# AMReX-Fluids/IAMR

Measured on AMD Instinct MI355X. Metric: cells-advanced/sec, higher is better.
Workload: dtype f64; 1 GPU; TaylorGreen 3D single level, one 256^3 box per GPU in a 1x1x1 arrangement (256x256x256 cells), periodic, nu=1e-4 cfl=0.7 Godunov_PLM be_cn_theta=0.5, full NavierStokes::advance per step

## Files before the change

iamr_amd/csrc/cabi.hip:

```cpp
#include "../../include/iamrx.h"
#include "operators.h"
#include "launch.h"
#include "amrns.h"
#include <string>
#include <cstring>
#include <vector>
#include <map>

using namespace iamrx;

struct iamrx_layout_s { LayoutP p; };
struct iamrx_mf_s { MultiFab mf; };

static thread_local std::string g_err;

#define IAMRX_TRY try {
#define IAMRX_CATCH                                                   \
    return 0; }                                                       \
    catch (const std::exception& e) { g_err = e.what(); return 1; }   \
    catch (...) { g_err = "unknown error"; return 2; }

static Geometry to_geom(const iamrx_geom* g)
{
    Geometry r;
// ... 452 lines not shown
            tb[d].define(phi->mf.layout, face_type(d), 3, 0);
            tensor_bcoef(tb[d], *b[d], d);
            b[d] = &tb[d];
        }
        mg.setTensor(true);
    }
    mg.setBCoeffs(b);
    mg.prepare();
    MGStats s = mg.solve(phi->mf, rhs->mf, rtol, atol);
    from_stats(s, st);
    IAMRX_CATCH
}

int iamrx_mlmg_mac_solve(const iamrx_geom* g, iamrx_mf ux, iamrx_mf uy, iamrx_mf uz, iamrx_mf rho, int rho_comp, iamrx_mf S,
                         iamrx_mf mac_phi, double rhs_scale, const int lobc[3], const int hibc[3], double mac_tol,
                         double mac_abs_tol, const iamrx_mg_opts* o, iamrx_mg_stats* st)
{
    IAMRX_TRY
    MGOpts op = to_opts(o);
    MultiFab* um[3] = {&ux->mf, &uy->mf, &uz->mf};
    MGStats s = mlmg_mac_solve(to_geom(g), um, rho->mf, rho_comp, S ? &S->mf : nullptr, mac_phi->mf, rhs_scale,
                               to_bc(lobc, hibc, op.maxorder), mac_tol, mac_abs_tol, op, nullptr);
    from_stats(s, st);
    IAMRX_CATCH
}

int iamrx_mlmg_mac_solve_cf(const iamrx_geom* g, iamrx_mf ux, iamrx_mf uy, iamrx_mf uz, iamrx_mf rho, int rho_comp, iamrx_mf S,
                            iamrx_mf mac_phi, double rhs_scale, const int lobc[3], const int hibc[3], iamrx_mf crse_phi,
                            const iamrx_geom* cgeom, int ratio, double mac_tol, double mac_abs_tol, const iamrx_mg_opts* o, iamrx_mg_stats* st)
{
    IAMRX_TRY
    IAMRX_ASSERT(ratio == 2 && cgeom);
    MGOpts op = to_opts(o);
    MultiFab* um[3] = {&ux->mf, &uy->mf, &uz->mf};
    const Geometry cg = to_geom(cgeom);
    MGStats s = mlmg_mac_solve(to_geom(g), um, rho->mf, rho_comp, S ? &S->mf : nullptr, mac_phi->mf, rhs_scale,
                               to_bc(lobc, hibc, op.maxorder), mac_tol, mac_abs_tol, op, nullptr, crse_phi ? &crse_phi->mf : nullptr, &cg, ratio);
    from_stats(s, st);
    IAMRX_CATCH
}

int iamrx_derive_mag_vort(const iamrx_geom* g, iamrx_mf out, int ocomp, iamrx_mf vel, int vcomp)
{
    IAMRX_TRY derive_mag_vort(to_geom(g), out->mf, ocomp, vel->mf, vcomp); IAMRX_CATCH
}

int iamrx_error_tag(const iamrx_geom* g, iamrx_mf tags, iamrx_mf field, int comp, int mode, double value, int level,
                    const double* realbox_lo, const double* realbox_hi)
{
    IAMRX_TRY error_tag(to_geom(g), tags->mf, field->mf, comp, mode, value, level, realbox_lo, realbox_hi); IAMRX_CATCH
}

int iamrx_host_cluster_tags(const unsigned char* tags, const int dom_lo[3], const int dom_hi[3], int blocking_factor, int max_grid_size, double grid_eff,
                            int n_error_buf, const unsigned char* allowed, int* boxes, int* nboxes)
{
    IAMRX_TRY
    BoxD dom;
    for (int d = 0; d < 3; ++d) { dom.lo[d] = dom_lo[d]; dom.hi[d] = dom_hi[d]; }
    std::vector<BoxD> bx = cluster_tags(tags, dom, blocking_factor, max_grid_size, grid_eff, n_error_buf, nullptr, allowed);
    if ((int)bx.size() > *nboxes) throw Error("iamrx_host_cluster_tags: box capacity too small");
    *nboxes = (int)bx.size();
    for (size_t q = 0; q < bx.size(); ++q) for (int d = 0; d < 3; ++d) { boxes[6 * q + d] = bx[q].lo[d]; boxes[6 * q + 3 + d] = bx[q].hi[d]; }
    IAMRX_CATCH
}
int iamrx_host_erode(unsigned char* map, const int n[3], const int periodic[3], int passes)
{
    IAMRX_TRY
    std::vector<unsigned char> m(map, map + (size_t)n[0] * n[1] * n[2]);
    int lo[3] = {n[0], n[1], n[2]}, hi[3] = {-1, -1, -1};
    for (int k = 0; k < n[2]; ++k) for (int j = 0; j < n[1]; ++j) for (int i = 0; i < n[0]; ++i)
        if (m[((size_t)k * n[1] + j) * n[0] + i]) { const int c[3] = {i, j, k}; for (int d = 0; d < 3; ++d) { lo[d] = std::min(lo[d], c[d]); hi[d] = std::max(hi[d], c[d]); } }
    erode_map(m, n, periodic, passes, lo, hi);
    std::copy(m.begin(), m.end(), map);
    IAMRX_CATCH
}
int iamrx_cluster_tags(const iamrx_geom* g, iamrx_mf tags, int blocking_factor, int max_grid_size, double grid_eff, int n_error_buf,
                       int* boxes, int* nboxes)
{
    IAMRX_TRY
    const Geometry gg = to_geom(g);
    const MultiFab& T = tags->mf;
    IAMRX_ASSERT(Context::get().comm->nranks == 1);
    const int n0 = gg.domain.len(0), n1 = gg.domain.len(1), n2 = gg.domain.len(2);
    std::vector<unsigned char> h((size_t)n0 * n1 * n2, 0);
    for (int li = 0; li < T.nlocal(); ++li) {
        const BoxD fb = T.fabbox(li);
        std::vector<double> buf((size_t)fb.npts() * T.ncomp);
        T.copy_to_host(li, buf.data());
        const BoxD vb = T.layout->lbox(li);
        for (int k = vb.lo[2]; k <= vb.hi[2]; ++k) for (int j = vb.lo[1]; j <= vb.hi[1]; ++j) for (int i = vb.lo[0]; i <= vb.hi[0]; ++i) {
            const size_t o = ((size_t)(k - fb.lo[2]) * fb.len(1) + (j - fb.lo[1])) * fb.len(0) + (i - fb.lo[0]);
            if (buf[o] != 0.0) h[((size_t)(k - gg.domain.lo[2]) * n1 + (j - gg.domain.lo[1])) * n0 + (i - gg.domain.lo[0])] = 1;
        }
    }
    std::vector<BoxD> bx = cluster_tags(h.data(), gg.domain, blocking_factor, max_grid_size, grid_eff, n_error_buf);
    if ((int)bx.size() > *nboxes) throw Error("iamrx_cluster_tags: box capacity too small");
    *nboxes = (int)bx.size();
    for (size_t q = 0; q < bx.size(); ++q) for (int d = 0; d < 3; ++d) { boxes[6 * q + d] = bx[q].lo[d]; boxes[6 * q + 3 + d] = bx[q].hi[d]; }
    IAMRX_CATCH
}

int iamrx_mac_divergence(const iamrx_geom* g, iamrx_mf div, iamrx_mf ux, iamrx_mf uy, iamrx_mf uz)
{
    IAMRX_TRY
    const MultiFab* um[3] = {&ux->mf, &uy->mf, &uz->mf};
    mac_divergence(to_geom(g), div->mf, um);
    IAMRX_CATCH
}

static std::vector<BCRec> to_bcrec(const int* b, int n)
{
    std::vector<BCRec> r(n);
    for (int i = 0; i < n; ++i)
        for (int d = 0; d < 3; ++d) { r[i].lo[d] = b ? b[6 * i + d] : 0; r[i].hi[d] = b ? b[6 * i + 3 + d] : 0; }
    return r;
}

int iamrx_mf_fill_physbc(iamrx_mf m, const iamrx_geom* g, int scomp, int ncomp, const int* bcrec, const double* edlo, const double* edhi)
{
    IAMRX_TRY
    auto bc = to_bcrec(bcrec, ncomp);
    fill_physbc_cc(to_geom(g), m->mf, scomp, ncomp, bc.data(), edlo, edhi);
    IAMRX_CATCH
}

int iamrx_godunov_extrap_vel_to_faces(const iamrx_geom* g, iamrx_mf vel, iamrx_mf force, iamrx_mf ux, iamrx_mf uy, iamrx_mf uz,
                                      double dt, const int* bcrec, int fit, int scheme)
{
    IAMRX_TRY
    auto bc = to_bcrec(bcrec, 3);
    MultiFab* um[3] = {&ux->mf, &uy->mf, &uz->mf};
    godunov_extrap_vel_to_faces(to_geom(g), vel->mf, force ? &force->mf : nullptr, um, dt, bc.data(), fit != 0, scheme);
    IAMRX_CATCH
}

int iamrx_godunov_compute_aofs(const iamrx_geom* g, iamrx_mf aofs, int acomp, iamrx_mf S, int ncomp, iamrx_mf force, iamrx_mf divu,
                               iamrx_mf ux, iamrx_mf uy, iamrx_mf uz, const int* iconserv, double dt, const int* bcrec,
                               int is_velocity, int fit, iamrx_mf ex, iamrx_mf ey, iamrx_mf ez, iamrx_mf fx, iamrx_mf fy, iamrx_mf fz, int scheme)
{
    IAMRX_TRY
    auto bc = to_bcrec(bcrec, ncomp);
    MultiFab* um[3] = {&ux->mf, &uy->mf, &uz->mf};
    MultiFab* ed[3] = {ex ? &ex->mf : nullptr, ey ? &ey->mf : nullptr, ez ? &ez->mf : nullptr};
    MultiFab* fl[3] = {fx ? &fx->mf : nullptr, fy ? &fy->mf : nullptr, fz ? &fz->mf : nullptr};
    godunov_compute_aofs(to_geom(g), aofs->mf, acomp, S->mf, ncomp, force ? &force->mf : nullptr, divu ? &divu->mf : nullptr, um,
                         iconserv, dt, bc.data(), is_velocity != 0, fit != 0, ex ? ed : nullptr, fx ? fl : nullptr, scheme);
    IAMRX_CATCH
}

int iamrx_nodal_residual(const iamrx_geom* g, iamrx_mf out, iamrx_mf phi, iamrx_mf sig, iamrx_mf rhs)
{
    IAMRX_TRY nodal_residual(to_geom(g), out->mf, phi->mf, sig->mf, rhs ? &rhs->mf : nullptr); IAMRX_CATCH
}
int iamrx_nodal_gs_color(const iamrx_geom* g, iamrx_mf phi, iamrx_mf rhs, iamrx_mf sig, int color)
{
    IAMRX_TRY nodal_gs_color(to_geom(g), phi->mf, rhs->mf, sig->mf, color); IAMRX_CATCH
}
int iamrx_nodal_gs_sweep(const iamrx_geom* g, iamrx_mf phi, iamrx_mf rhs, iamrx_mf sig, int fused)
{
    IAMRX_TRY
    Geometry gg = to_geom(g);
    if (fused == 3 || fused == 4) {
        static MultiFab& xb = *new MultiFab();
        if (!xb.defined() || xb.layout != phi->mf.layout || xb.ngrow != phi->mf.ngrow) xb.define(phi->mf.layout, node_type(), 1, phi->mf.ngrow);
        const bool wrap = fused == 4;
        if (wrap && !periodic_wrap_ok(gg, *phi->mf.layout, 4)) throw Error("iamrx_nodal_gs_sweep(4): not a single box spanning a periodic domain");
        const double cs = tune("BENCH_CSIG", 0.0);
        nodal_gs_fused_pass(gg, phi->mf, phi->mf, xb, rhs->mf, sig->mf, 0, wrap, nullptr, cs != 0.0 ? &cs : nullptr);
        nodal_gs_fused_pass(gg, phi->mf, xb, xb, rhs->mf, sig->mf, 1, wrap, nullptr, cs != 0.0 ? &cs : nullptr);
    } else if (fused == 2) {
        if (!nodal_smooth_small(gg, phi->mf, rhs->mf, sig->mf, 1)) throw Error("level does not qualify for the single-workgroup smoother");
        phi->mf.FillBoundary(gg);
    } else if (fused) {
        MultiFab xb(phi->mf.layout, node_type(), 1, phi->mf.ngrow);
        phi->mf.FillBoundary(gg);
        nodal_gs_fused_pass(gg, phi->mf, phi->mf, xb, rhs->mf, sig->mf, 0);
        xb.FillBoundary(gg);
        nodal_gs_fused_pass(gg, phi->mf, xb, xb, rhs->mf, sig->mf, 1);
        MultiFab::Copy(phi->mf, xb, 0, 0, 1, 0);
    } else {
        for (int c = 0; c < 8; ++c) { phi->mf.FillBoundary(gg); nodal_gs_color(gg, phi->mf, rhs->mf, sig->mf, c); }
    }
    IAMRX_CATCH
}
int iamrx_nodal_restrict(iamrx_mf c, iamrx_mf f) { IAMRX_TRY nodal_restrict(c->mf, f->mf); IAMRX_CATCH }
int iamrx_nodal_interp_add(iamrx_mf f, iamrx_mf c, iamrx_mf s) { IAMRX_TRY nodal_interp_add(f->mf, c->mf, s->mf); IAMRX_CATCH }
int iamrx_nodal_divu(const iamrx_geom* g, iamrx_mf rhs, iamrx_mf vel, int vcomp)
{
    IAMRX_TRY
    Geometry gg = to_geom(g);
    DomainBC bc;
    for (int d = 0; d < 3; ++d) bc.lo[d] = bc.hi[d] = gg.periodic[d] ? lo_periodic : lo_neumann;
    bc.maxorder = 2;
    nodal_divu(gg, rhs->mf, vel->mf, vcomp, &bc);
    IAMRX_CATCH
}
int iamrx_nodal_divu_bc(const iamrx_geom* g, iamrx_mf rhs, iamrx_mf vel, int vcomp, const int lobc[3], const int hibc[3])
{
    IAMRX_TRY
    const DomainBC bc = to_bc(lobc, hibc, 2);
    nodal_divu(to_geom(g), rhs->mf, vel->mf, vcomp, &bc);
    IAMRX_CATCH
}
int iamrx_nodal_compgrad(const iamrx_geom* g, iamrx_mf gp, iamrx_mf phi)
{
    IAMRX_TRY nodal_mknewu(to_geom(g), nullptr, 0, phi->mf, nullptr, &gp->mf, false); IAMRX_CATCH
}

int iamrx_nodal_projection(const iamrx_geom* g, iamrx_mf vel, int vcomp, iamrx_mf phi, iamrx_mf sig, int sig_comp, const int lobc[3],
                           const int hibc[3], double rel_tol, double abs_tol, const iamrx_mg_opts* o, iamrx_mf gp, int increment_gp,
                           iamrx_mg_stats* st)
{
    IAMRX_TRY
    MGOpts op = to_opts(o);
    MGStats s = nodal_projection(to_geom(g), vel->mf, vcomp, phi->mf, sig->mf, sig_comp, to_bc(lobc, hibc, op.maxorder), rel_tol, abs_tol,
                                 op, gp ? &gp->mf : nullptr, increment_gp != 0);
    from_stats(s, st);
    IAMRX_CATCH
}

int iamrx_nodal_solve(const iamrx_geom* g, iamrx_mf phi, iamrx_mf rhs, iamrx_mf sig, int sig_comp, const int lobc[3], const int hibc[3],
                      double rel_tol, double abs_tol, const iamrx_mg_opts* o, iamrx_mg_stats* st)
{
    IAMRX_TRY
    MGOpts op = to_opts(o);
    NodalMG mg(to_geom(g), phi->mf.layout, to_bc(lobc, hibc, op.maxorder), op);
    mg.setSigma(sig->mf, sig_comp);
    MGStats s = mg.solve(phi->mf, rhs->mf, rel_tol, abs_tol);
    from_stats(s, st);
    IAMRX_CATCH
}

int iamrx_tensor_apply(const iamrx_geom* g, iamrx_mf out, iamrx_mf vel, double a, double b, iamrx_mf acoef, iamrx_mf ex, iamrx_mf ey,
                       iamrx_mf ez, const int* lobc, const int* hibc, int nbc, int maxorder)
{
    IAMRX_TRY
    IAMRX_ASSERT(nbc == 1 || nbc == 3);
    const MultiFab* eta[3] = {&ex->mf, &ey->mf, &ez->mf};
    DomainBC bcs[3];
    for (int n = 0; n < nbc; ++n) bcs[n] = to_bc(lobc + 3 * n, hibc + 3 * n, maxorder);
    tensor_apply(to_geom(g), out->mf, vel->mf, a, b, acoef ? &acoef->mf : nullptr, eta, bcs, nbc);
    IAMRX_CATCH
}

int iamrx_tensor_solve(const iamrx_geom* g, iamrx_mf soln, iamrx_mf rhs, double a, double b, iamrx_mf acoef, iamrx_mf ex, iamrx_mf ey,
                       iamrx_mf ez, const int* lobc, const int* hibc, int nbc, double tol_rel, double tol_abs, const iamrx_mg_opts* o,
                       iamrx_mg_stats* st)
{
    IAMRX_TRY
    IAMRX_ASSERT(nbc == 1 || nbc == 3);
    MGOpts op = to_opts(o);
    const MultiFab* eta[3] = {&ex->mf, &ey->mf, &ez->mf};
    DomainBC bcs[3];
    for (int n = 0; n < nbc; ++n) bcs[n] = to_bc(lobc + 3 * n, hibc + 3 * n, op.maxorder);
    MGStats s = tensor_solve(to_geom(g), soln->mf, rhs->mf, a, b, acoef ? &acoef->mf : nullptr, eta, bcs, nbc, tol_rel, tol_abs, op);
    from_stats(s, st);
    IAMRX_CATCH
}

int iamrx_tensor_extensive_flux(const iamrx_geom* g, iamrx_mf vel, iamrx_mf ex, iamrx_mf ey, iamrx_mf ez, iamrx_mf fx, iamrx_mf fy, iamrx_mf fz,
                                double fac, int add)
{
    IAMRX_TRY
    const MultiFab* eta[3] = {&ex->mf, &ey->mf, &ez->mf};
    MultiFab* fl[3] = {&fx->mf, &fy->mf, &fz->mf};
    tensor_extensive_flux(to_geom(g), vel->mf, eta, fl, fac, add != 0);
    IAMRX_CATCH
}

int iamrx_tensor_apply_cf(const iamrx_geom* g, iamrx_mf out, iamrx_mf vel, double a, double b, iamrx_mf acoef, iamrx_mf ex, iamrx_mf ey,
                          iamrx_mf ez, const int* lobc, const int* hibc, int nbc, int maxorder, iamrx_mf crse_vel, const iamrx_geom* cgeom, int ratio)
{
    IAMRX_TRY
    IAMRX_ASSERT(nbc == 1 || nbc == 3);
    const MultiFab* eta[3] = {&ex->mf, &ey->mf, &ez->mf};
    DomainBC bcs[3];
    for (int n = 0; n < nbc; ++n) bcs[n] = to_bc(lobc + 3 * n, hibc + 3 * n, maxorder);
    Geometry cg = to_geom(cgeom);
    TensorCF cf{crse_vel ? &crse_vel->mf : nullptr, &cg, ratio};
    tensor_apply(to_geom(g), out->mf, vel->mf, a, b, acoef ? &acoef->mf : nullptr, eta, bcs, nbc, &cf);
    IAMRX_CATCH
}

int iamrx_tensor_solve_cf(const iamrx_geom* g, iamrx_mf soln, iamrx_mf rhs, double a, double b, iamrx_mf acoef, iamrx_mf ex, iamrx_mf ey,
                          iamrx_mf ez, const int* lobc, const int* hibc, int nbc, iamrx_mf crse_vel, const iamrx_geom* cgeom, int ratio,
                          double tol_rel, double tol_abs, const iamrx_mg_opts* o, iamrx_mg_stats* st)
{
    IAMRX_TRY
    IAMRX_ASSERT(nbc == 1 || nbc == 3);
    MGOpts op = to_opts(o);
    const MultiFab* eta[3] = {&ex->mf, &ey->mf, &ez->mf};
    DomainBC bcs[3];
    for (int n = 0; n < nbc; ++n) bcs[n] = to_bc(lobc + 3 * n, hibc + 3 * n, op.maxorder);
    Geometry cg = to_geom(cgeom);
    TensorCF cf{crse_vel ? &crse_vel->mf : nullptr, &cg, ratio};
    MGStats s = tensor_solve(to_geom(g), soln->mf, rhs->mf, a, b, acoef ? &acoef->mf : nullptr, eta, bcs, nbc, tol_rel, tol_abs, op, &cf);
    from_stats(s, st);
    IAMRX_CATCH
}

int iamrx_les_mut(const iamrx_geom* g, iamrx_mf vel, int vcomp, int model, double Cs, double base, iamrx_mf mu_x, iamrx_mf mu_y, iamrx_mf mu_z)
{
    IAMRX_TRY
    MultiFab* mu[3] = {&mu_x->mf, &mu_y->mf, &mu_z->mf};
    les_mut(to_geom(g), vel->mf, vcomp, model, Cs, base, mu);
    IAMRX_CATCH
// ... 824 lines not shown
```

iamr_amd/csrc/k_nodal.hip:

```cpp
#include "kernels.h"
#include <cstring>
#include <type_traits>
#include "launch.h"

namespace iamrx {

struct NodeW { double corner, ex, ey, ez, fx, fy, fz, c; };

static NodeW make_w(const Geometry& g)
{
    const double fx = 1.0 / (g.dx[0] * g.dx[0]) / 36.0, fy = 1.0 / (g.dx[1] * g.dx[1]) / 36.0, fz = 1.0 / (g.dx[2] * g.dx[2]) / 36.0;
    NodeW w;
    w.corner = fx + fy + fz;
    w.ex = -fx + 2.0 * fy + 2.0 * fz;
    w.ey = 2.0 * fx - fy + 2.0 * fz;
    w.ez = 2.0 * fx + 2.0 * fy - fz;
    w.fx = 4.0 * fx - 2.0 * fy - 2.0 * fz;
    w.fy = -2.0 * fx + 4.0 * fy - 2.0 * fz;
    w.fz = -2.0 * fx - 2.0 * fy + 4.0 * fz;
    w.c = -4.0 * (fx + fy + fz);
    return w;
}

__device__ __forceinline__ double node_Ax(const FabD& x, const FabD& s, const NodeW& w, int i, int j, int k, double& s0)
{
    const double smmm = s(i - 1, j - 1, k - 1), spmm = s(i, j - 1, k - 1), smpm = s(i - 1, j, k - 1), sppm = s(i, j, k - 1);
    const double smmp = s(i - 1, j - 1, k), spmp = s(i, j - 1, k), smpp = s(i - 1, j, k), sppp = s(i, j, k);
    s0 = w.c * (smmm + spmm + smpm + sppm + smmp + spmp + smpp + sppp);
    double y = x(i, j, k) * s0;
    y += w.corner * (x(i - 1, j - 1, k - 1) * smmm + x(i + 1, j - 1, k - 1) * spmm + x(i - 1, j + 1, k - 1) * smpm + x(i + 1, j + 1, k - 1) * sppm
                   + x(i - 1, j - 1, k + 1) * smmp + x(i + 1, j - 1, k + 1) * spmp + x(i - 1, j + 1, k + 1) * smpp + x(i + 1, j + 1, k + 1) * sppp);
    y += w.ex * (x(i, j - 1, k - 1) * (smmm + spmm) + x(i, j + 1, k - 1) * (smpm + sppm) + x(i, j - 1, k + 1) * (smmp + spmp) + x(i, j + 1, k + 1) * (smpp + sppp));
    y += w.ey * (x(i - 1, j, k - 1) * (smmm + smpm) + x(i + 1, j, k - 1) * (spmm + sppm) + x(i - 1, j, k + 1) * (smmp + smpp) + x(i + 1, j, k + 1) * (spmp + sppp));
    y += w.ez * (x(i - 1, j - 1, k) * (smmm + smmp) + x(i + 1, j - 1, k) * (spmm + spmp) + x(i - 1, j + 1, k) * (smpm + smpp) + x(i + 1, j + 1, k) * (sppm + sppp));
    y += w.fx * (x(i - 1, j, k) * (smmm + smpm + smmp + smpp) + x(i + 1, j, k) * (spmm + sppm + spmp + sppp));
    y += w.fy * (x(i, j - 1, k) * (smmm + spmm + smmp + spmp) + x(i, j + 1, k) * (smpm + sppm + smpp + sppp));
    y += w.fz * (x(i, j, k - 1) * (smmm + spmm + smpm + sppm) + x(i, j, k + 1) * (smmp + spmp + smpp + sppp));
    return y;
}

void nodal_residual_launch(const Geometry& g, MultiFab& out, const MultiFab& x, const MultiFab& sig, const MultiFab* rhs, unsigned long long* d_norm);
__device__ __forceinline__ void nodal_norm_commit(double mx, unsigned long long* out)
{
    for (int o = 32; o > 0; o >>= 1) mx = fmax(mx, __shfl_xor(mx, o, 64));
    if ((threadIdx.x & 63) == 0 && mx > 0.0) {
        const unsigned long long bits = (unsigned long long)__double_as_longlong(mx);
        if (bits > __atomic_load_n(out, __ATOMIC_RELAXED)) atomicMax(out, bits);
    }
}
template <int TX, int TY>
__global__ void __launch_bounds__(TX * TY) k_nodal_residual_zm(const BoxD* __restrict__ boxes, const FabD* __restrict__ ot, const FabD* __restrict__ xt,
    const FabD* __restrict__ st, const FabD* __restrict__ rt, NodeW w, int ntx, int nty, int kc, unsigned long long* __restrict__ normout,
    const int4* __restrict__ list)
{
    double mx = 0.0;
    constexpr int RX = TX + 2, RY = TY + 2, NT = TX * TY, NLD = (RX * RY + NT - 1) / NT;
    __shared__ double X[3][RY][RX];
    __shared__ double S[2][RY][RX];
    int fab = blockIdx.y, tix, tiy, ck;
    if (list) { const int4 e = list[blockIdx.x]; fab = e.x; tix = e.y; tiy = e.z; ck = e.w; }
    else { const int bid = blockIdx.x; tix = bid % ntx; const int r1 = bid / ntx; tiy = r1 % nty; ck = r1 / nty; }
    const BoxD cb = boxes[fab];
    const int nhi0 = cb.hi[0] + 1, nhi1 = cb.hi[1] + 1, nhi2 = cb.hi[2] + 1;
    const int tx0 = cb.lo[0] + tix * TX, ty0 = cb.lo[1] + tiy * TY, k0 = cb.lo[2] + ck * kc;
    if (tx0 > nhi0 || ty0 > nhi1 || k0 > nhi2) return;
    const int k1 = min(k0 + kc - 1, nhi2);
    const FabD x = xt[fab], s = st[fab], o = ot[fab];
    const int ox = tx0 - 1, oy = ty0 - 1;
    const int tid = threadIdx.x;
    long xoff[NLD], soff[NLD];
    int lidx[NLD];
#pragma unroll
    for (int it = 0; it < NLD; ++it) {
        const int idx = min(tid + it * NT, RX * RY - 1);
        lidx[it] = idx;
        const int gi = ox + idx % RX, gj = oy + idx / RX;
        const int xi = min(max(gi, x.lo[0]), x.lo[0] + x.n[0] - 1), xj = min(max(gj, x.lo[1]), x.lo[1] + x.n[1] - 1);
        const int si = min(max(gi, s.lo[0]), s.lo[0] + s.n[0] - 1), sj = min(max(gj, s.lo[1]), s.lo[1] + s.n[1] - 1);
        xoff[it] = x.off(xi, xj, x.lo[2]);
        soff[it] = s.off(si, sj, s.lo[2]);
    }
    const long xpl = (long)x.n[0] * x.n[1], spl = (long)s.n[0] * s.n[1];
    const FabD::gdouble* xp = (const FabD::gdouble*)x.p;
    const FabD::gdouble* sp = (const FabD::gdouble*)s.p;
    auto ldx = [&](int it, int k) { return xp[xoff[it] + xpl * (k - x.lo[2])]; };
    auto lds_ = [&](int it, int k) { return sp[soff[it] + spl * (k - s.lo[2])]; };
#pragma unroll
    for (int it = 0; it < NLD; ++it) {
        const int ly = lidx[it] / RX, lx = lidx[it] % RX;
        X[(k0 + 2) % 3][ly][lx] = ldx(it, k0 - 1);
        X[k0 % 3][ly][lx] = ldx(it, k0);
        S[(k0 + 1) & 1][ly][lx] = lds_(it, k0 - 1);
    }
    double vx[NLD], vs[NLD];
#pragma unroll
    for (int it = 0; it < NLD; ++it) { vx[it] = ldx(it, k0 + 1); vs[it] = lds_(it, k0); }
    const int lx = tid % TX + 1, ly = tid / TX + 1;
    const int i = ox + lx, j = oy + ly;
    const bool valid = i <= nhi0 && j <= nhi1;
    for (int k = k0; k <= k1; ++k) {
        const int a0 = (k + 2) % 3, a1 = k % 3, a2 = (k + 1) % 3, b0 = (k + 1) & 1, b1 = k & 1;
#pragma unroll
        for (int it = 0; it < NLD; ++it) {
            const int qy = lidx[it] / RX, qx = lidx[it] % RX;
            X[a2][qy][qx] = vx[it];
            S[b1][qy][qx] = vs[it];
        }
        __syncthreads();
        if (k < k1) {
#pragma unroll
            for (int it = 0; it < NLD; ++it) { vx[it] = ldx(it, k + 2); vs[it] = lds_(it, k + 1); }
        }
        if (valid) {
            const double smmm = S[b0][ly - 1][lx - 1], spmm = S[b0][ly - 1][lx], smpm = S[b0][ly][lx - 1], sppm = S[b0][ly][lx];
            const double smmp = S[b1][ly - 1][lx - 1], spmp = S[b1][ly - 1][lx], smpp = S[b1][ly][lx - 1], sppp = S[b1][ly][lx];
            const double s0 = w.c * (smmm + spmm + smpm + sppm + smmp + spmp + smpp + sppp);
            double y = X[a1][ly][lx] * s0;
            y += w.corner * (X[a0][ly - 1][lx - 1] * smmm + X[a0][ly - 1][lx + 1] * spmm + X[a0][ly + 1][lx - 1] * smpm + X[a0][ly + 1][lx + 1] * sppm
                           + X[a2][ly - 1][lx - 1] * smmp + X[a2][ly - 1][lx + 1] * spmp + X[a2][ly + 1][lx - 1] * smpp + X[a2][ly + 1][lx + 1] * sppp);
            y += w.ex * (X[a0][ly - 1][lx] * (smmm + spmm) + X[a0][ly + 1][lx] * (smpm + sppm) + X[a2][ly - 1][lx] * (smmp + spmp) + X[a2][ly + 1][lx] * (smpp + sppp));
            y += w.ey * (X[a0][ly][lx - 1] * (smmm + smpm) + X[a0][ly][lx + 1] * (spmm + sppm) + X[a2][ly][lx - 1] * (smmp + smpp) + X[a2][ly][lx + 1] * (spmp + sppp));
            y += w.ez * (X[a1][ly - 1][lx - 1] * (smmm + smmp) + X[a1][ly - 1][lx + 1] * (spmm + spmp) + X[a1][ly + 1][lx - 1] * (smpm + smpp) + X[a1][ly + 1][lx + 1] * (sppm + sppp));
            y += w.fx * (X[a1][ly][lx - 1] * (smmm + smpm + smmp + smpp) + X[a1][ly][lx + 1] * (spmm + sppm + spmp + sppp));
            y += w.fy * (X[a1][ly - 1][lx] * (smmm + spmm + smmp + spmp) + X[a1][ly + 1][lx] * (smpm + sppm + smpp + sppp));
            y += w.fz * (X[a0][ly][lx] * (smmm + spmm + smpm + sppm) + X[a2][ly][lx] * (smmp + spmp + smpp + sppp));
            const double v = rt ? rt[fab](i, j, k) - y : y;
            o(i, j, k) = v;
            const double a = fabs(v);
            mx = fmax(mx, a == a ? a : INFINITY);
        }
        __syncthreads();
    }
    if (normout) nodal_norm_commit(mx, normout);
}

bool nodal_residual(const Geometry& g, MultiFab& out, const MultiFab& x, const MultiFab& sig, const MultiFab* rhs, double* norm_out)
{
    auto& ctx = Context::get();
    static unsigned long long* d_norm = nullptr;
    if (norm_out && !d_norm) IAMRX_HIP_CHECK(hipMalloc(&d_norm, 2 * sizeof(unsigned long long)));
    const Layout& lay = *x.layout;
    const bool zm = tune("NODAL_RES_ZM", 1) != 0 && lay.max_len[0] >= 16 && lay.max_len[1] >= 8 && x.ngrow >= 1 && sig.ngrow >= 1;
    const bool fused = norm_out && zm && tune("NODAL_RES_NORM", 1) != 0;
    if (fused) IAMRX_HIP_CHECK(hipMemsetAsync(d_norm, 0, sizeof(unsigned long long), ctx.stream));
    nodal_residual_launch(g, out, x, sig, rhs, fused ? d_norm : nullptr);
    if (!fused) return false;
    const bool global = !lay.replicated && ctx.comm->nranks > 1;
    if (global) ctx.comm->allreduce_device(reinterpret_cast<double*>(d_norm), 1, ReduceOp::Max, ctx.stream);
    unsigned long long bits = 0;
    IAMRX_HIP_CHECK(hipMemcpyAsync(&bits, d_norm, sizeof(bits), hipMemcpyDeviceToHost, ctx.stream));
    ctx.sync();
    double v;
    std::memcpy(&v, &bits, sizeof(v));
    *norm_out = v;
    return true;
}

void nodal_residual_launch(const Geometry& g, MultiFab& out, const MultiFab& x, const MultiFab& sig, const MultiFab* rhs, unsigned long long* d_norm)
{
    if (x.nlocal() == 0) return;
    const NodeW w = make_w(g);
    const FabD *ot = out.d_tab, *xt = x.d_tab, *st = sig.d_tab;
    const FabD* rt = rhs ? rhs->d_tab : nullptr;
    const Layout& l = *x.layout;
    const bool zmarch = tune("NODAL_RES_ZM", 1) != 0;
    if (zmarch && l.max_len[0] >= 16 && l.max_len[1] >= 8 && x.ngrow >= 1 && sig.ngrow >= 1) {
        constexpr int TX = 32, TY = 8;
        const int ntx = (l.max_len[0] + 1 + TX - 1) / TX, nty = (l.max_len[1] + 1 + TY - 1) / TY;
        const int nk = l.max_len[2] + 1;
        const int kc = nk >= 128 ? 32 : (nk >= 32 ? 16 : nk);
        const int nck = (nk + kc - 1) / kc;
        if (l.nlocal() >= 4 && tune("TILE_LISTS", 1) != 0) {
            int n = 0;
            const int4* lst = layout_int4_list(l, {3, TX, TY, kc, 0}, [&](std::vector<int4>& h) {
                for (int f = 0; f < l.nlocal(); ++f) {
                    const BoxD b = l.lbox(f);
                    const int bx = (b.len(0) + 1 + TX - 1) / TX, by = (b.len(1) + 1 + TY - 1) / TY, bk = (b.len(2) + 1 + kc - 1) / kc;
                    for (int c = 0; c < bk; ++c) for (int ty = 0; ty < by; ++ty) for (int tx = 0; tx < bx; ++tx) h.push_back(make_int4(f, tx, ty, c));
                }
            }, &n);
            if (lst && 4L * n <= 3L * ntx * nty * nck * l.nlocal()) {
                hipLaunchKernelGGL((k_nodal_residual_zm<TX, TY>), dim3((unsigned)n), dim3(TX * TY), 0, Context::get().stream, l.d_boxes, ot, xt, st, rt, w, ntx, nty, kc,
                                   d_norm, lst);
                return;
            }
        }
        dim3 grid((unsigned)(ntx * nty * nck), (unsigned)l.nlocal());
        hipLaunchKernelGGL((k_nodal_residual_zm<TX, TY>), grid, dim3(TX * TY), 0, Context::get().stream, l.d_boxes, ot, xt, st, rt, w, ntx, nty, kc, d_norm,
                           (const int4*)nullptr);
        return;
    }
    for_each(*x.layout, node_type(), 0, Context::get().stream, [=] __device__(int i, int j, int k, int f) {
        double s0;
        const double y = node_Ax(xt[f], st[f], w, i, j, k, s0);
        ot[f](i, j, k) = rt ? rt[f](i, j, k) - y : y;
    });
}

__global__ void __launch_bounds__(256) k_nodal_gscolor(Tiling t, const BoxD* __restrict__ boxes, const FabD* __restrict__ xt,
    const FabD* __restrict__ rt, const FabD* __restrict__ st, NodeW w, int color, const FabD* __restrict__ dmt)
{
    const int fab = blockIdx.y;
    const BoxD cb = boxes[fab];
    const int cx = color & 1, cy = (color >> 1) & 1, cz = (color >> 2) & 1;
    const int i0 = cb.lo[0] + (((cb.lo[0] & 1) != cx) ? 1 : 0);
    const int j0 = cb.lo[1] + (((cb.lo[1] & 1) != cy) ? 1 : 0);
    const int k0n = cb.lo[2] + (((cb.lo[2] & 1) != cz) ? 1 : 0);
    BoxD hb;
    hb.lo[0] = hb.lo[1] = hb.lo[2] = 0;
    hb.hi[0] = (cb.hi[0] + 1 - i0) >> 1; hb.hi[1] = (cb.hi[1] + 1 - j0) >> 1; hb.hi[2] = (cb.hi[2] + 1 - k0n) >> 1;
    if (cb.hi[0] + 1 < i0 || cb.hi[1] + 1 < j0 || cb.hi[2] + 1 < k0n) return;
    int mi, mj, mk0, mk1;
    if (!tile_ijk(t, hb, mi, mj, mk0, mk1)) return;
    const FabD x = xt[fab], r = rt[fab], s = st[fab];
    const int i = i0 + 2 * mi, j = j0 + 2 * mj;
    for (int mk = mk0; mk <= mk1; ++mk) {
        const int k = k0n + 2 * mk;
        if (dmt && dmt[fab](i, j, k) != 0.0) continue;
        double s0;
        const double Ax = node_Ax(x, s, w, i, j, k, s0);
        x(i, j, k) += (r(i, j, k) - Ax) / s0;
    }
}

void nodal_gs_color(const Geometry& g, MultiFab& x, const MultiFab& rhs, const MultiFab& sig, int color, const MultiFab* dmask)
{
    if (x.nlocal() == 0) return;
    const Layout& l = *x.layout;
    int ml[3];
    for (int d = 0; d < 3; ++d) ml[d] = (l.max_len[d] + 1 + 1) / 2;
    Tiling t = make_tiling(ml, l.nlocal(), 4);
    hipLaunchKernelGGL(k_nodal_gscolor, t.grid(), Tiling::block(), 0, Context::get().stream, t, l.d_boxes, x.d_tab, rhs.d_tab, sig.d_tab, make_w(g), color,
                       dmask ? dmask->d_tab : nullptr);
}

__device__ __forceinline__ int wrap_node(int g, int lo, int hi)
{
    const int n = hi - lo + 1;
    return g < lo ? g + n : (g > hi + 1 ? g - n : g);
}
__device__ __forceinline__ int wrap_cell(int g, int lo, int hi)
{
    const int n = hi - lo + 1;
    return g < lo ? g + n : (g > hi ? g - n : g);
}
__device__ __forceinline__ int image_node(int g, int lo, int hi, bool refl)
{
    if (refl) return g < lo ? 2 * lo - g : (g > hi + 1 ? 2 * (hi + 1) - g : g);
    return wrap_node(g, lo, hi);
}
__device__ __forceinline__ int image_cell(int g, int lo, int hi, bool refl)
{
    if (refl) return g < lo ? 2 * lo - 1 - g : (g > hi ? 2 * hi + 1 - g : g);
    return wrap_cell(g, lo, hi);
}

template <int TX, int TY, int NT, bool WRAP, bool MASK, bool CSIG>
__global__ void __launch_bounds__(NT, (MASK && NT == 256 ? 3 : 1)) k_nodal_gs4(const BoxD* __restrict__ boxes, const FabD* __restrict__ xct, const FabD* __restrict__ xnt,
    const FabD* __restrict__ xot, const FabD* __restrict__ rt, const FabD* __restrict__ st, NodeW w, int kpar, int ntx, int nty, int xcd_chunk,
    const FabD* __restrict__ dmt, double csig, int ppc, int refl)
{
    constexpr int RX = TX + 8, RY = TY + 8, HX = RX / 2, PX = RX + 2;
    constexpr int PL = RY * PX;
    __shared__ double Xf[3 * PL];
    __shared__ double Sf[CSIG ? 1 : 2 * PL];
    const int fab = blockIdx.y;
    const BoxD cb = boxes[fab];
    int tix, tiy, pk;
    if (xcd_chunk > 0) {
        const int q = blockIdx.x & 7, m = blockIdx.x >> 3;
        const int nt = ntx * nty;
        const int tlo = (q * nt) >> 3, cnt = (((q + 1) * nt) >> 3) - tlo;
        if (cnt == 0 || m >= cnt * xcd_chunk) return;
        const int t = tlo + m % cnt;
        pk = m / cnt;
        tix = t % ntx; tiy = t / ntx;
    } else {
        const int bid = blockIdx.x;
        tix = bid % ntx;
        const int r1 = bid / ntx;
        tiy = r1 % nty; pk = r1 / nty;
    }
    const int kfirst = cb.lo[2] + (((cb.lo[2] & 1) != kpar) ? 1 : 0);
    const int k0 = kfirst + 2 * pk * ppc;
    const int nhi0 = cb.hi[0] + 1, nhi1 = cb.hi[1] + 1, nhi2 = cb.hi[2] + 1;
    const int tx0 = cb.lo[0] + tix * TX, ty0 = cb.lo[1] + tiy * TY;
    if (k0 > nhi2 || tx0 > nhi0 || ty0 > nhi1) return;
    const int kend = min(k0 + 2 * (ppc - 1), nhi2);
    const int txe = min(tx0 + TX - 1, nhi0), tye = min(ty0 + TY - 1, nhi1);
    const FabD x = xct[fab], xn = xnt[fab], xo = xot[fab], r = rt[fab], s = st[fab];
    const int ox = tx0 - 4, oy = ty0 - 4;
    const int tid = threadIdx.x;
#define COL(lx) ((((lx) & 1) * HX) + ((lx) >> 1))
    static_assert(((TX + 7) / 2) * ((TY + 7) / 2) <= NT, "one node per thread and colour pass");
    int q0[4], qm[4];
    int roff[4], doff[4];
    double rr[4];
    bool fixed[4];
    bool surf[4];
    const int rks = r.n[0] * r.n[1];
    int dks = 0;
    if constexpr (MASK) dks = dmt[fab].n[0] * dmt[fab].n[1];
#pragma unroll
    for (int c = 0; c < 4; ++c) {
        const int cx = c & 1, cy = c >> 1, g = 3 - c;
        const int rlo0 = tx0 - g, rhi0 = txe + g, rlo1 = ty0 - g, rhi1 = tye + g;
        const int i0 = rlo0 + (((rlo0 & 1) != cx) ? 1 : 0), j0 = rlo1 + (((rlo1 & 1) != cy) ? 1 : 0);
        const int ni = i0 > rhi0 ? 0 : ((rhi0 - i0) >> 1) + 1, nj = j0 > rhi1 ? 0 : ((rhi1 - j0) >> 1) + 1;
        const bool on = tid < ni * nj;
        const int pi = i0 + 2 * (tid % max(ni, 1)), pj = j0 + 2 * (tid / max(ni, 1));
        const int lx = pi - ox, ly = pj - oy;
        q0[c] = on ? ly * PX + COL(lx) : -1;
        qm[c] = ly * PX + COL(lx - 1);
        int ri = on ? pi : tx0, rj = on ? pj : ty0;
        if constexpr (WRAP) { ri = image_node(ri, cb.lo[0], cb.hi[0], refl & 1); rj = image_node(rj, cb.lo[1], cb.hi[1], refl & 2); }
        roff[c] = (int)r.off(ri, rj, r.lo[2]);
        rr[c] = r.gp()[roff[c] + (long)(k0 - r.lo[2]) * rks];
        if constexpr (MASK) {
            doff[c] = (int)dmt[fab].off(ri, rj, dmt[fab].lo[2]);
            surf[c] = ri <= cb.lo[0] || ri >= nhi0 || rj <= cb.lo[1] || rj >= nhi1;
            fixed[c] = (surf[c] || k0 <= cb.lo[2] || k0 >= nhi2) ? dmt[fab].gp()[doff[c] + (long)(k0 - dmt[fab].lo[2]) * dks] != 0.0 : false;
        } else { doff[c] = 0; fixed[c] = false; surf[c] = false; }
    }
    constexpr int NLD = (RX * RY + NT - 1) / NT;
    int xoff[NLD], soff[NLD];
    int lslot[NLD];
    const int xks = x.n[0] * x.n[1], sks = s.n[0] * s.n[1];
#pragma unroll
    for (int it = 0; it < NLD; ++it) {
        const int idx = min(tid + it * NT, RX * RY - 1);
        const int lx = idx % RX, ly = idx / RX;
        const int gi = ox + lx, gj = oy + ly;
        int xi, xj, si, sj;
        if constexpr (WRAP) {
            xi = image_node(gi, cb.lo[0], cb.hi[0], refl & 1); xj = image_node(gj, cb.lo[1], cb.hi[1], refl & 2);
            si = image_cell(gi, cb.lo[0], cb.hi[0], refl & 1); sj = image_cell(gj, cb.lo[1], cb.hi[1], refl & 2);
        } else {
            xi = min(max(gi, x.lo[0]), x.lo[0] + x.n[0] - 1); xj = min(max(gj, x.lo[1]), x.lo[1] + x.n[1] - 1);
            si = min(max(gi, s.lo[0]), s.lo[0] + s.n[0] - 1); sj = min(max(gj, s.lo[1]), s.lo[1] + s.n[1] - 1);
        }
        xoff[it] = (int)x.off(xi, xj, x.lo[2]);
        soff[it] = CSIG ? 0 : (int)s.off(si, sj, s.lo[2]);
        lslot[it] = (tid + it * NT < RX * RY) ? ly * PX + COL(lx) : -1;
    }
    auto xk = [&](int kk) -> long { if constexpr (WRAP) kk = image_node(kk, cb.lo[2], cb.hi[2], refl & 4); return (long)(kk - x.lo[2]) * xks; };
    auto sk = [&](int kk) -> long { if constexpr (WRAP) kk = image_cell(kk, cb.lo[2], cb.hi[2], refl & 4); return (long)(kk - s.lo[2]) * sks; };
    double* Xm = Xf;
    double* Xc = Xf + PL;
    double* Xp = Xf + 2 * PL;
    {
        double v[NLD][CSIG ? 3 : 5];
        const auto *pm = xn.gp() + xk(k0 - 1), *pc = x.gp() + xk(k0), *pp = xn.gp() + xk(k0 + 1);
        const auto *ps0 = s.gp() + sk(k0 - 1), *ps1 = s.gp() + sk(k0);
#pragma unroll
        for (int it = 0; it < NLD; ++it) {
            v[it][0] = pm[xoff[it]];
            v[it][1] = pc[xoff[it]];
            v[it][2] = pp[xoff[it]];
            if constexpr (!CSIG) { v[it][3] = ps0[soff[it]]; v[it][4] = ps1[soff[it]]; }
        }
#pragma unroll
        for (int it = 0; it < NLD; ++it) {
            if (lslot[it] >= 0) {
                Xm[lslot[it]] = v[it][0]; Xc[lslot[it]] = v[it][1]; Xp[lslot[it]] = v[it][2];
                if constexpr (!CSIG) { Sf[lslot[it]] = v[it][3]; Sf[PL + lslot[it]] = v[it][4]; }
            }
        }
    }
    const int wx = txe - tx0 + 1, wy = tye - ty0 + 1;
    for (int k = k0;; k += 2) {
        const bool has_next = k + 2 <= kend;
        double nv[NLD][CSIG ? 2 : 4], rrn[4];
        bool fixedn[4];
        if (has_next) {
            const auto *pc = x.gp() + xk(k + 2), *pp = xn.gp() + xk(k + 3);
            const auto *ps0 = s.gp() + sk(k + 1), *ps1 = s.gp() + sk(k + 2);
#pragma unroll
            for (int it = 0; it < NLD; ++it) {
                nv[it][0] = pc[xoff[it]];
                nv[it][1] = pp[xoff[it]];
                if constexpr (!CSIG) { nv[it][2] = ps0[soff[it]]; nv[it][3] = ps1[soff[it]]; }
            }
            const auto* pr = r.gp() + (long)(k + 2 - r.lo[2]) * rks;
#pragma unroll
            for (int c = 0; c < 4; ++c) {
                rrn[c] = pr[roff[c]];
                if constexpr (MASK)
                    fixedn[c] = (surf[c] || k + 2 <= cb.lo[2] || k + 2 >= nhi2) ? dmt[fab].gp()[doff[c] + (long)(k + 2 - dmt[fab].lo[2]) * dks] != 0.0 : false;
                else fixedn[c] = false;
            }
        }
        __syncthreads();
#pragma unroll
        for (int c = 0; c < 4; ++c) {
            if (q0[c] >= 0 && !(MASK && fixed[c])) {
                const int a0 = q0[c], am = qm[c], ap = am + 1;
                double smmm, spmm, smpm, sppm, smmp, spmp, smpp, sppp;
                if constexpr (CSIG) { smmm = spmm = smpm = sppm = smmp = spmp = smpp = sppp = csig; }
                else {
                    smmm = Sf[am - PX]; spmm = Sf[a0 - PX]; smpm = Sf[am]; sppm = Sf[a0];
                    smmp = Sf[PL + am - PX]; spmp = Sf[PL + a0 - PX]; smpp = Sf[PL + am]; sppp = Sf[PL + a0];
                }
                const double s0 = w.c * (smmm + spmm + smpm + sppm + smmp + spmp + smpp + sppp);
                const double xc = Xc[a0];
                double y = xc * s0;
                y += w.corner * (Xm[am - PX] * smmm + Xm[ap - PX] * spmm + Xm[am + PX] * smpm + Xm[ap + PX] * sppm
                               + Xp[am - PX] * smmp + Xp[ap - PX] * spmp + Xp[am + PX] * smpp + Xp[ap + PX] * sppp);
// ... 849 lines not shown
    };
    const double rhs0 = on ? (double)res(i, j, k) : 0.0;
    double bb = rhs0;
    if (singular) bb -= nbg_sum(wt * rhs0, red) / mean_cnt;
    if (!on) bb = 0.0;
    double x = 0.0, r = bb, p = 0.0, v = 0.0;
    const double rh = r;
    const double rnorm0 = nbg_max(fabs(r), red);
    double rnorm = rnorm0;
    int ret = 0, nit = 0;
    if (rnorm0 != 0.0) {
        double rho_1 = 0.0, alph = 0.0, omg = 0.0;
        for (nit = 1; nit <= maxiter; ++nit) {
            const double rho = nbg_sum(wt * rh * r, red);
            if (rho == 0.0) { ret = 1; break; }
            if (nit == 1) p = r;
            else {
                const double beta = (rho / rho_1) * (alph / omg);
                p = p - omg * v;
                p = r + beta * p;
            }
            v = apply(p);
            const double rhTv = nbg_sum(wt * rh * v, red);
            if (rhTv != 0.0) alph = rho / rhTv; else { ret = 2; break; }
            x = x + alph * p;
            const double sv = r - alph * v;
            rnorm = nbg_max(fabs(sv), red);
            if (rnorm < eps_rel * rnorm0) break;
            const double t = apply(sv);
            const double tt = nbg_sum(wt * t * t, red), ts = nbg_sum(wt * t * sv, red);
            if (tt != 0.0) omg = ts / tt; else { ret = 3; break; }
            x = x + omg * sv;
            r = sv - omg * t;
            rnorm = nbg_max(fabs(r), red);
            if (rnorm < eps_rel * rnorm0) break;
            if (omg == 0.0) { ret = 4; break; }
            rho_1 = rho;
        }
        if (ret == 0 && rnorm > eps_rel * rnorm0) ret = 8;
        if (!((ret == 0 || ret == 8) && rnorm < rnorm0)) x = 0.0;
    }
    if (tid == 0 && iters_out) atomicAdd(iters_out, nit);
    int ncalls = ret == 0 ? nub : nuf;
    if (ret != 0) { x = 0.0; ncalls += nuf; }
    __syncthreads();
    if (in) V[tid] = x;
    __syncthreads();
    for (int sw = 0; sw < ncalls * nsweeps; ++sw)
        for (int c = 0; c < 8; ++c) {
            const int cx = c & 1, cy = (c >> 1) & 1, cz = (c >> 2) & 1;
            if (on && (i & 1) == cx && (j & 1) == cy && (k & 1) == cz) {
                x += (rhs0 - Ax()) / s0;
                V[tid] = x;
            }
            __syncthreads();
        }
    const int f0 = G.n[0] + 1, f1 = G.n[1] + 1, f2 = G.n[2] + 1;
    for (int q = tid; q < f0 * f1 * f2; q += NBG_NT) {
        const int qi = q % f0, qq = q / f0, qj = qq % f1, qk = qq / f1;
        const int a = (G.wrap[0] && qi == G.n[0]) ? 0 : qi, b = (G.wrap[1] && qj == G.n[1]) ? 0 : qj, c = (G.wrap[2] && qk == G.n[2]) ? 0 : qk;
        cor(G.lo[0] + qi, G.lo[1] + qj, G.lo[2] + qk) = V[a + m0 * (b + m1 * c)];
    }
}

static bool nbg_geom(const Geometry& g, const Layout& l, NBotGeom& G)
{
    if (l.boxes.size() != 1) return false;
    const BoxD& b = l.boxes[0];
    long M = 1;
    for (int d = 0; d < 3; ++d) {
        if (b.len(d) < 2 || b.len(d) > 8) return false;
        G.wrap[d] = (g.periodic[d] && b.lo[d] == g.domain.lo[d] && b.hi[d] == g.domain.hi[d]) ? 1 : 0;
        G.m[d] = b.len(d) + (G.wrap[d] ? 0 : 1);
        G.lo[d] = b.lo[d]; G.n[d] = b.len(d);
        G.half_lo[d] = g.half_lo[d]; G.half_hi[d] = g.half_hi[d]; G.dlo[d] = g.domain.lo[d]; G.dhi[d] = g.domain.hi[d];
        M *= G.m[d];
    }
    return M <= NBG_NT;
}

bool nodal_bottom_device_ok_general(const Geometry& g, const Layout& l)
{
    const bool enabled = tune("MG_DEVICE_BOTTOM", 1) != 0 && tune("MG_DEVICE_BOTTOM_GENERAL", 1) != 0;
    NBotGeom G;
    return enabled && nbg_geom(g, l, G);
}

void nodal_bottom_solve_general(const Geometry& g, MultiFab& cor, const MultiFab& res, const MultiFab& sig, const MultiFab* dmask, bool singular,
                                double eps_rel, int maxiter, int nsweeps, int nub, int nuf, int* d_iters)
{
    const Layout& l = *cor.layout;
    NBotGeom G;
    IAMRX_ASSERT(nbg_geom(g, l, G) && sig.ngrow >= 1);
    if (l.nlocal() == 0) return;
    double cnt = 1.0;
    for (int d = 0; d < 3; ++d) cnt *= (double)g.domain.len(d);
    hipLaunchKernelGGL(k_nodal_bottom_g, dim3(1), dim3(NBG_NT), 0, Context::get().stream, cor.d_tab, res.d_tab, sig.d_tab,
                       dmask ? dmask->d_tab : nullptr, make_w(g), G, singular ? 1 : 0, cnt, eps_rel, maxiter, nsweeps, nub, nuf, d_iters);
}

void nodal_jacobi(const Geometry& g, MultiFab& xnew, const MultiFab& x, const MultiFab& rhs, const MultiFab& sig, const MultiFab* dmask)
{
    if (x.nlocal() == 0) return;
    const NodeW w = make_w(g);
    const FabD *nt = xnew.d_tab, *xt = x.d_tab, *rt = rhs.d_tab, *st = sig.d_tab, *dt = dmask ? dmask->d_tab : nullptr;
    for_each(*x.layout, node_type(), 0, Context::get().stream, [=] __device__(int i, int j, int k, int f) {
        if (dt && dt[f](i, j, k) != 0.0) { nt[f](i, j, k) = xt[f](i, j, k); return; }
        double s0;
        const double Ax = node_Ax(xt[f], st[f], w, i, j, k, s0);
        nt[f](i, j, k) = xt[f](i, j, k) + (2. / 3.) * (rt[f](i, j, k) - Ax) / s0;
    });
}

void nodal_zero_masked(MultiFab& mf, const MultiFab& dmask)
{
    if (mf.nlocal() == 0) return;
    const FabD *mt = mf.d_tab, *dt = dmask.d_tab;
    for_each(*mf.layout, node_type(), 0, Context::get().stream, [=] __device__(int i, int j, int k, int f) {
        if (dt[f](i, j, k) != 0.0) mt[f](i, j, k) = 0.0;
    });
}

void nodal_build_dmask(const Geometry& g, MultiFab& dm, const MultiFab& cov, const DomainBC& bc)
{
    if (dm.nlocal() == 0) return;
    const FabD *dt = dm.d_tab, *ct = cov.d_tab;
    int lo[3], hi[3], tlo[3], thi[3];
    for (int d = 0; d < 3; ++d) {
        lo[d] = g.domain.lo[d]; hi[d] = g.domain.hi[d];
        tlo[d] = g.periodic[d] ? 0 : bc.lo[d]; thi[d] = g.periodic[d] ? 0 : bc.hi[d];
    }
    const int l0 = lo[0], l1 = lo[1], l2 = lo[2], h0 = hi[0], h1 = hi[1], h2 = hi[2];
    const int a0 = tlo[0], a1 = tlo[1], a2 = tlo[2], b0 = thi[0], b1 = thi[1], b2 = thi[2];
    for_each(*dm.layout, node_type(), 0, Context::get().stream, [=] __device__(int i, int j, int k, int f) {
        const FabD c = ct[f];
        bool in = true;
        for (int q = 0; q < 8; ++q) {
            int ci = i - 1 + (q & 1), cj = j - 1 + ((q >> 1) & 1), ck = k - 1 + ((q >> 2) & 1);
            bool out = false;
            if (ci < l0) { if (a0 == lo_neumann) ci = 2 * l0 - 1 - ci; else if (a0 != 0) out = true; }
            else if (ci > h0) { if (b0 == lo_neumann) ci = 2 * h0 + 1 - ci; else if (b0 != 0) out = true; }
            if (cj < l1) { if (a1 == lo_neumann) cj = 2 * l1 - 1 - cj; else if (a1 != 0) out = true; }
            else if (cj > h1) { if (b1 == lo_neumann) cj = 2 * h1 + 1 - cj; else if (b1 != 0) out = true; }
            if (ck < l2) { if (a2 == lo_neumann) ck = 2 * l2 - 1 - ck; else if (a2 != 0) out = true; }
            else if (ck > h2) { if (b2 == lo_neumann) ck = 2 * h2 + 1 - ck; else if (b2 != 0) out = true; }
            if (out || c(ci, cj, ck) == 0.0) in = false;
        }
        dt[f](i, j, k) = in ? 0.0 : 1.0;
    });
}

template <int CTX, int CTY>
__global__ void __launch_bounds__(CTX * CTY) k_nodal_restrict_tile(const BoxD* __restrict__ cboxes, const FabD* __restrict__ ct, const FabD* __restrict__ ft,
    int ntx, int nty, int kc)
{
    constexpr int FX = 2 * CTX + 1, FY = 2 * CTY + 1, HX = CTX + 1, PX = 2 * HX, NT = CTX * CTY, NLD = (FX * FY + NT - 1) / NT;
    __shared__ double F[3][FY][PX];
    const int fab = blockIdx.y;
    const BoxD cb = cboxes[fab];
    const int bid = blockIdx.x;
    const int tix = bid % ntx, r1 = bid / ntx, tiy = r1 % nty, ck = r1 / nty;
    const int nhi0 = cb.hi[0] + 1, nhi1 = cb.hi[1] + 1, nhi2 = cb.hi[2] + 1;
    const int i0 = cb.lo[0] + tix * CTX, j0 = cb.lo[1] + tiy * CTY, k0 = cb.lo[2] + ck * kc;
    if (i0 > nhi0 || j0 > nhi1 || k0 > nhi2) return;
    const int k1 = min(k0 + kc - 1, nhi2);
    const FabD fa = ft[fab], c = ct[fab];
    const int ox = 2 * i0 - 1, oy = 2 * j0 - 1;
    const int tid = threadIdx.x;
    long foff[NLD];
    int lslot[NLD];
    const int fhi0 = min(2 * nhi0 + 1, fa.lo[0] + fa.n[0] - 1), fhi1 = min(2 * nhi1 + 1, fa.lo[1] + fa.n[1] - 1);
#pragma unroll
    for (int it = 0; it < NLD; ++it) {
        const int idx = tid + it * NT;
        const int lx = idx % FX, ly = idx / FX;
        const int gi = ox + lx, gj = oy + ly;
        const bool on = idx < FX * FY && gi >= fa.lo[0] && gi <= fhi0 && gj >= fa.lo[1] && gj <= fhi1;
        foff[it] = on ? fa.off(gi, gj, fa.lo[2]) : -1;
        lslot[it] = idx < FX * FY ? ly * PX + (lx & 1) * HX + (lx >> 1) : -1;
    }
    const long fpl = (long)fa.n[0] * fa.n[1];
    const FabD::gdouble* fp = (const FabD::gdouble*)fa.p;
    const int fklo = fa.lo[2], fkhi = fa.lo[2] + fa.n[2] - 1;
    auto ldf = [&](int it, int k) { return (foff[it] >= 0 && k >= fklo && k <= fkhi) ? (double)fp[foff[it] + fpl * (k - fklo)] : 0.0; };
    double* Fl = &F[0][0][0];
    constexpr int PL = FY * PX;
    int sm = 0, s0 = 1, sp = 2;
    double v0[NLD], v1[NLD];
#pragma unroll
    for (int it = 0; it < NLD; ++it) {
        const double vm = ldf(it, 2 * k0 - 1);
        v0[it] = ldf(it, 2 * k0); v1[it] = ldf(it, 2 * k0 + 1);
        if (lslot[it] >= 0) Fl[sm * PL + lslot[it]] = vm;
    }
    const int tx = tid % CTX, ty = tid / CTX;
    const int i = i0 + tx, j = j0 + ty;
    const bool valid = i <= nhi0 && j <= nhi1;
    const int cxm = tx, cx0 = HX + tx, cxp = tx + 1;
    for (int k = k0; k <= k1; ++k) {
#pragma unroll
        for (int it = 0; it < NLD; ++it)
            if (lslot[it] >= 0) { Fl[s0 * PL + lslot[it]] = v0[it]; Fl[sp * PL + lslot[it]] = v1[it]; }
        __syncthreads();
        if (k < k1) {
#pragma unroll
            for (int it = 0; it < NLD; ++it) { v0[it] = ldf(it, 2 * k + 2); v1[it] = ldf(it, 2 * k + 3); }
        }
        if (valid) {
            const int pl[3] = {sm, s0, sp};
            double s = 0.0;
#pragma unroll
            for (int dk = 0; dk < 3; ++dk)
#pragma unroll
                for (int dj = 0; dj < 3; ++dj) {
                    const double* row = Fl + pl[dk] * PL + (2 * ty + dj) * PX;
                    const double wjk = (dj == 1 ? 2. : 1.) * (dk == 1 ? 2. : 1.);
                    s += (1. * wjk) * row[cxm];
                    s += (2. * wjk) * row[cx0];
                    s += (1. * wjk) * row[cxp];
                }
            c(i, j, k) = s * (1. / 64.);
        }
        __syncthreads();
        const int t = sm; sm = sp; sp = s0; s0 = t;
    }
}

void nodal_restrict(MultiFab& crse, const MultiFab& fine)
{
    if (crse.nlocal() == 0) return;
    const FabD *ct = crse.d_tab, *ft = fine.d_tab;
    const Layout& cl = *crse.layout;
    const int min_x = std::max(16, (int)tune("NODAL_RESTRICT_MIN", 48));
    if (tune("NODAL_RESTRICT_TILE", 1) != 0 && cl.max_len[0] >= min_x && cl.max_len[1] >= 8 && fine.ngrow >= 1) {
        constexpr int CTX = 32, CTY = 8;
        const int ntx = (cl.max_len[0] + 1 + CTX - 1) / CTX, nty = (cl.max_len[1] + 1 + CTY - 1) / CTY;
        const int nk = cl.max_len[2] + 1;
        const int kc = nk >= 64 ? 8 : 4;
        const int nck = (nk + kc - 1) / kc;
        dim3 grid((unsigned)(ntx * nty * nck), (unsigned)cl.nlocal());
        hipLaunchKernelGGL((k_nodal_restrict_tile<CTX, CTY>), grid, dim3(CTX * CTY), 0, Context::get().stream, cl.d_boxes, ct, ft, ntx, nty, kc);
        return;
    }
    for_each(*crse.layout, node_type(), 0, Context::get().stream, [=] __device__(int i, int j, int k, int f) {
        const FabD fa = ft[f];
        const int ii = 2 * i, jj = 2 * j, kk = 2 * k;
        double s = 0.0;
        for (int dk = -1; dk <= 1; ++dk)
            for (int dj = -1; dj <= 1; ++dj)
                for (int di = -1; di <= 1; ++di) {
                    const double w = (di == 0 ? 2. : 1.) * (dj == 0 ? 2. : 1.) * (dk == 0 ? 2. : 1.);
                    s += w * fa(ii + di, jj + dj, kk + dk);
                }
        ct[f](i, j, k) = s * (1. / 64.);
    });
}

#ifndef IAMRX_INTERP_EXP
#define IAMRX_INTERP_EXP 0
#endif
__device__ __forceinline__ double w_side(const FabD& s, int i, int j, int k, int d, int side)
{
    int lo[3] = {i - 1, j - 1, k - 1}, hi[3] = {i, j, k};
    lo[d] = hi[d] = (d == 0 ? i : (d == 1 ? j : k)) - 1 + side;
    double r = 0.0;
    for (int c = lo[2]; c <= hi[2]; ++c) for (int b = lo[1]; b <= hi[1]; ++b) for (int a = lo[0]; a <= hi[0]; ++a) r += s(a, b, c);
    return r;
}
__device__ __forceinline__ double interp_line(const FabD& c, const FabD& s, int i, int j, int k, int ic, int jc, int kc, int d)
{
    const double w1 = w_side(s, i, j, k, d, 0), w2 = w_side(s, i, j, k, d, 1);
    const double c2 = c(ic + (d == 0), jc + (d == 1), kc + (d == 2));
    return (c(ic, jc, kc) * w1 + c2 * w2) / (w1 + w2);
}
__device__ __forceinline__ double interp_face(const FabD& c, const FabD& s, int i, int j, int k, int ic, int jc, int kc, int d1, int d2)
{
    const double w1 = w_side(s, i, j, k, d1, 0), w2 = w_side(s, i, j, k, d1, 1), w3 = w_side(s, i, j, k, d2, 0), w4 = w_side(s, i, j, k, d2, 1);
    const int e1[3] = {d1 == 0, d1 == 1, d1 == 2}, e2[3] = {d2 == 0, d2 == 1, d2 == 2};
    double r = 0.0;
    r += w1 * interp_line(c, s, i - e1[0], j - e1[1], k - e1[2], ic, jc, kc, d2);
    r += w2 * interp_line(c, s, i + e1[0], j + e1[1], k + e1[2], ic + e1[0], jc + e1[1], kc + e1[2], d2);
    r += w3 * interp_line(c, s, i - e2[0], j - e2[1], k - e2[2], ic, jc, kc, d1);
    r += w4 * interp_line(c, s, i + e2[0], j + e2[1], k + e2[2], ic + e2[0], jc + e2[1], kc + e2[2], d1);
    return r / (w1 + w2 + w3 + w4);
}

template <class SA>
__device__ __forceinline__ void side_weights(const SA& s, int i, int j, int k, double w[6])
{
#if IAMRX_INTERP_EXP & 1
    for (int t = 0; t < 6; ++t) w[t] = 1.0 + 1e-3 * t;
    return;
#endif
    double g[2][2][2];
#pragma unroll
    for (int c = 0; c < 2; ++c)
#pragma unroll
        for (int b = 0; b < 2; ++b)
#pragma unroll
            for (int a = 0; a < 2; ++a) g[c][b][a] = s(i - 1 + a, j - 1 + b, k - 1 + c);
#pragma unroll
    for (int t = 0; t < 2; ++t) {
        w[t] = ((g[0][0][t] + g[0][1][t]) + g[1][0][t]) + g[1][1][t];
        w[2 + t] = ((g[0][t][0] + g[0][t][1]) + g[1][t][0]) + g[1][t][1];
        w[4 + t] = ((g[t][0][0] + g[t][0][1]) + g[t][1][0]) + g[t][1][1];
    }
}

template <int PX, int PY, int PZ, int CX, int CY, int CZ, class SA>
__device__ __forceinline__ void interp_class(double (*T)[2 * CY + 1][2 * CX + 1], const FabD& c, const SA& s, int fi0, int fj0, int fk0,
                                             int nhi0, int nhi1, int nhi2, int tid)
{
    constexpr int NX = PX ? CX : CX + 1, NY = PY ? CY : CY + 1, NZ = PZ ? CZ : CZ + 1, CLS = PX + PY + PZ;
    for (int idx = tid; idx < NX * NY * NZ; idx += 256) {
        const int lx = 2 * (idx % NX) + PX, q = idx / NX, ly = 2 * (q % NY) + PY, lz = 2 * (q / NY) + PZ;
        const int i = fi0 + lx, j = fj0 + ly, k = fk0 + lz;
        if (i > nhi0 || j > nhi1 || k > nhi2) continue;
        if (CLS == 0) { T[lz][ly][lx] = c(i >> 1, j >> 1, k >> 1); continue; }
        double w[6];
        side_weights(s, i, j, k, w);
        if (CLS == 1) {
            constexpr int d = PX ? 0 : (PY ? 1 : 2);
            const double w1 = w[2 * d], w2 = w[2 * d + 1];
            T[lz][ly][lx] = (IAMRX_INTERP_EXP & 4) ? (T[lz - PZ][ly - PY][lx - PX] * w1 + T[lz + PZ][ly + PY][lx + PX] * w2) * (w1 + w2) : (T[lz - PZ][ly - PY][lx - PX] * w1 + T[lz + PZ][ly + PY][lx + PX] * w2) / (w1 + w2);
        } else if (CLS == 2) {
            constexpr int d1 = PX ? 0 : 1, d2 = PZ ? 2 : 1;
            constexpr int ax = d1 == 0, ay = d1 == 1, by = d2 == 1, bz = d2 == 2;
            const double w1 = w[2 * d1], w2 = w[2 * d1 + 1], w3 = w[2 * d2], w4 = w[2 * d2 + 1];
            double r = 0.0;
            r += w1 * T[lz][ly - ay][lx - ax];
            r += w2 * T[lz][ly + ay][lx + ax];
            r += w3 * T[lz - bz][ly - by][lx];
            r += w4 * T[lz + bz][ly + by][lx];
            T[lz][ly][lx] = (IAMRX_INTERP_EXP & 4) ? r * (w1 + w2 + w3 + w4) : r / (w1 + w2 + w3 + w4);
        } else {
            T[lz][ly][lx] = (w[0] * T[lz][ly][lx - 1] + w[1] * T[lz][ly][lx + 1] + w[2] * T[lz][ly - 1][lx] + w[3] * T[lz][ly + 1][lx]
                             + w[4] * T[lz - 1][ly][lx] + w[5] * T[lz + 1][ly][lx]) / (w[0] + w[1] + w[2] + w[3] + w[4] + w[5]);
        }
    }
}

template <int CX, int CY, int CZ>
__global__ void __launch_bounds__(256) k_nodal_interp_lds(const BoxD* __restrict__ fboxes, const FabD* __restrict__ ft, const FabD* __restrict__ ct,
    const FabD* __restrict__ st, int ntx, int nty)
{
    constexpr int FX = 2 * CX + 1, FY = 2 * CY + 1, FZ = 2 * CZ + 1, NF = FX * FY * FZ;
    __shared__ double T[FZ][FY][FX];
    const int fab = blockIdx.y;
    const BoxD vb = fboxes[fab];
    const int bid = blockIdx.x;
    const int tix = bid % ntx, r1 = bid / ntx, tiy = r1 % nty, tiz = r1 / nty;
    const int nhi0 = vb.hi[0] + 1, nhi1 = vb.hi[1] + 1, nhi2 = vb.hi[2] + 1;
    const int fi0 = vb.lo[0] + tix * 2 * CX, fj0 = vb.lo[1] + tiy * 2 * CY, fk0 = vb.lo[2] + tiz * 2 * CZ;
    if (fi0 >= nhi0 || fj0 >= nhi1 || fk0 >= nhi2) return;
    const FabD c = ct[fab], sg = st[fab], fa = ft[fab];
    const int tid = threadIdx.x;
    const FabD& s = sg;
#define IAMRX_ICLS(PX, PY, PZ) interp_class<PX, PY, PZ, CX, CY, CZ>(T, c, s, fi0, fj0, fk0, nhi0, nhi1, nhi2, tid)
    IAMRX_ICLS(0, 0, 0);
    __syncthreads();
    IAMRX_ICLS(1, 0, 0); IAMRX_ICLS(0, 1, 0); IAMRX_ICLS(0, 0, 1);
    __syncthreads();
    IAMRX_ICLS(1, 1, 0); IAMRX_ICLS(1, 0, 1); IAMRX_ICLS(0, 1, 1);
    __syncthreads();
    IAMRX_ICLS(1, 1, 1);
    __syncthreads();
#undef IAMRX_ICLS
    for (int idx = tid; idx < NF; idx += 256) {
        const int lx = idx % FX, q = idx / FX, ly = q % FY, lz = q / FY;
        const int i = fi0 + lx, j = fj0 + ly, k = fk0 + lz;
        if (i > nhi0 || j > nhi1 || k > nhi2) continue;
        if ((lx == 2 * CX && i != nhi0) || (ly == 2 * CY && j != nhi1) || (lz == 2 * CZ && k != nhi2)) continue;
        if (IAMRX_INTERP_EXP & 2) fa(i, j, k) = T[lz][ly][lx]; else fa(i, j, k) += T[lz][ly][lx];
    }
}

static bool nodal_interp_lds_enabled()
{
    const bool on = tune("NODAL_INTERP_LDS", 1) != 0;
    return on;
}

void nodal_interp_add(MultiFab& fine, const MultiFab& crse, const MultiFab& sig_fine)
{
    if (fine.nlocal() == 0) return;
    if (nodal_interp_lds_enabled()) {
        const Layout& l = *fine.layout;
        bool even = true;
        for (int d = 0; d < 3; ++d) even = even && l.all_lo_even[d];
        if (even) {
            constexpr int CX = 16, CY = 4, CZ = 4;
            const int ntx = (l.max_len[0] + 2 * CX - 1) / (2 * CX), nty = (l.max_len[1] + 2 * CY - 1) / (2 * CY), ntz = (l.max_len[2] + 2 * CZ - 1) / (2 * CZ);
            dim3 grid((unsigned)(ntx * nty * ntz), (unsigned)l.nlocal());
            hipLaunchKernelGGL((k_nodal_interp_lds<CX, CY, CZ>), grid, dim3(256), 0, Context::get().stream, l.d_boxes, fine.d_tab, crse.d_tab, sig_fine.d_tab, ntx, nty);
            return;
        }
    }
    const FabD *ft = fine.d_tab, *ct = crse.d_tab, *st = sig_fine.d_tab;
    const BoxD* fb = fine.layout->d_boxes;
    for_each(*crse.layout, node_type(), 0, Context::get().stream, [=] __device__(int ic, int jc, int kc, int f) {
        const FabD c = ct[f], s = st[f], fa = ft[f];
        const BoxD vb = fb[f];
        const int nhi0 = vb.hi[0] + 1, nhi1 = vb.hi[1] + 1, nhi2 = vb.hi[2] + 1;
        const int i0 = 2 * ic, j0 = 2 * jc, k0 = 2 * kc;
        const bool xi = i0 + 1 <= nhi0, xj = j0 + 1 <= nhi1, xk = k0 + 1 <= nhi2;
// ... 187 lines not shown
```

iamr_amd/csrc/kernels.h:

```cpp
#pragma once
#include "core.h"
#include "mf.h"

namespace iamrx {

void launch_fill(double* p, size_t n, double v, hipStream_t s);
void launch_copy_plan(const CopyDesc* d, int nd, long maxpts, const FabD* src, const FabD* dst, int scomp, int dcomp, int nc, hipStream_t s, bool add = false);
void launch_pack(const CopyDesc* d, int nd, long maxpts, const FabD* src, double* buf, long pts_total, int scomp, int nc, hipStream_t s);
void launch_unpack(const CopyDesc* d, int nd, long maxpts, const FabD* dst, const double* buf, long pts_total, int dcomp, int nc, hipStream_t s, bool add = false);
void launch_copy_plan_w(const CopyDesc* d, const int2* w, int nw, const FabD* src, const FabD* dst, int scomp, int dcomp, int nc, hipStream_t s, bool add);
void launch_pack_w(const CopyDesc* d, const int2* w, int nw, const FabD* src, double* buf, long pts_total, int scomp, int nc, hipStream_t s);
void launch_unpack_w(const CopyDesc* d, const int2* w, int nw, const FabD* dst, const double* buf, long pts_total, int dcomp, int nc, hipStream_t s, bool add);
double reduce_norm0(const MultiFab& mf, int comp, int nc, int ng, bool global = false);
void reduce_norm0_comps(const MultiFab& mf, int comp, int nc, int ng, double* out, bool global = false);
void reduce_minmax(const MultiFab& mf, int comp, int ng, double& mn, double& mx, bool global = true);
double reduce_sum_unique(const MultiFab& mf, int comp, const Geometry& g, bool global = false);
void reduce_sum_integrated(const MultiFab& S, int rho_comp, int trac_comp, const MultiFab* cov, double out[3]);
void reduce_dots(int nout, const MultiFab* const* x, const MultiFab* const* y, int comp, int nc, const Geometry& g, double* out, bool local = false);
void reduce_dots_dev(int nout, const MultiFab* const* x, const MultiFab* const* y, int comp, int nc, const Geometry& g, double* d_out, bool local = false);
enum { PROBE_NODAL_GS4 = 0, PROBE_ABEC_GSRB = 1, PROBE_GOD_Z = 2, PROBE_PRED_Z = 3, PROBE_COUNT = 4 };
void kernel_probe_start(int which, long min_points, int stride);
void kernel_probe_stop(int which, double* total_ms, long* launches);
void kernel_probes_pause(bool on);
bool kernel_probe_begin(int which, long points);
void kernel_probe_end(int which);
void gs4_probe_start(long min_nodes, int stride);
void gs4_probe_stop(double* total_ms, long* launches);
void mf_lincomb(MultiFab& dst, double a, const MultiFab& x, double b, const MultiFab& y, int comp, int nc, int ng);
void mf_saxpy(MultiFab& y, double a, const MultiFab& x, int xcomp, int ycomp, int nc, int ng);
void mf_add_scalar(MultiFab& y, double a, int comp, int nc, int ng);
void mf_mult(MultiFab& y, double a, int comp, int nc, int ng);
void mf_mult_ghosts(MultiFab& y, double a, int comp, int nc, int ng);

void stats_accumulate(MultiFab& avg, const MultiFab& S, int vcomp, double dt_avg, double t_sum, bool fluct);
void stats_derive_vel_avg(MultiFab& out, int ocomp, const MultiFab& avg, double t_mean, double t_fluct);

struct DomainBC;
void fill_physbc_cc(const Geometry& g, MultiFab& mf, int scomp, int ncomp, const BCRec* bc, const double* extdir_lo, const double* extdir_hi);

void nodal_reflect_bc(const Geometry& g, MultiFab& mf, const DomainBC& bc, hipStream_t on = nullptr);
void cc_mirror_bc(const Geometry& g, MultiFab& mf);

struct AbecCoef {
    double alpha, beta;
    const MultiFab* a;
    const MultiFab* b[3];
    int tensor;
    int tensor_eta = 0;
    const MultiFab* sig = nullptr;
    int sig_comp = 0;
    double sig_scale = 1.0;
    int b_uniform = 0;
    double bu[3] = {0.0, 0.0, 0.0};
};
bool mf_uniform_value(const MultiFab& m, double* v);
bool tensor_residual_fused(const Geometry& g, const AbecCoef& c, MultiFab& out, const MultiFab& vel, const MultiFab* rhs, double* norm_out);
struct DomainBC {
    int lo[3], hi[3];
    int maxorder;
};
struct CfTab { double c[3][3][4]; int maxorder; };
CfTab cf_make_tab(const double loc[3], const double dx[3], int maxorder);
void cf_build_mask(const Geometry& g, MultiFab& cfm);
void cf_fill_ghosts(MultiFab& phi, const MultiFab& cfm, const CfTab& tab, bool inhomog, const MultiFab* bcval, bool edges = false);
void cf_interp_edges(MultiFab& bcval, const MultiFab& cpatch, const MultiFab& cfm, int ratio, const Geometry& cgeom);
void cf_interp_bndry(MultiFab& bcval, const MultiFab& cpatch, const MultiFab& cfm, int ratio);
struct AbecLevel {
    const std::vector<BoxD>* boxes = nullptr;
    int nlocal = 0, max_len[3] = {0, 0, 0};
    int ncomp = 1;
    int phi_ngrow = 1, rhs_ngrow = 0, sig_ngrow = 0, a_ngrow = 0;
    bool sig = false, b_uniform = false, has_a = false, tensor_eta = false;
    bool tensor = false;
    int b_ncomp = 1;
    int nbc = 0;
    const DomainBC* bcs = nullptr;
    bool has_cf = false;
    bool finest = true;
};
AbecLevel abec_level(const AbecCoef& c, const MultiFab& phi, int rhs_ngrow, int nbc, const DomainBC* bcs, bool has_cf = false, bool finest = true);
struct AbecColourForm {
    enum Kernel { GENERAL, GSRB1, GSRB2, GSRB2_PER_COMP } kernel = GENERAL;
    int mode = 0;
    int np = 1;
    bool gen_mc = false;
    int gen_mode = 0;
    bool has_cf = false, maintain = false, allcf = false;
    bool wrap = false;
    bool walls_inkernel = false;
    bool zero_ok = false;
};
struct AbecSmoothPlan {
    enum Path { COLOUR, RB_BOX, RB_CF, RB_NBR, FUSED_SHELL } path = COLOUR;
    AbecColourForm colour;
    int nw = 16;
    bool nbr_splits = false;
    bool zero_first = false;
    int ncomp = 1, phi_ngrow = 1, rhs_ngrow = 0;
    bool sweep_kernel() const { return path == RB_BOX || path == RB_CF || path == RB_NBR; }
    bool made_for(const MultiFab& phi, const MultiFab& rhs) const { return phi.ncomp == ncomp && phi.ngrow == phi_ngrow && rhs.ngrow == rhs_ngrow; }
};
AbecSmoothPlan abec_smooth_plan(const Geometry& g, const AbecLevel& lv);
AbecColourForm abec_colour_form(const Geometry& g, const AbecLevel& lv, bool wrap = false, bool walls_inkernel = false);
void abec_gsrb(const Geometry& g, const AbecCoef& c, const AbecColourForm& f, MultiFab& phi, const MultiFab& rhs, int redblack, double omega,
               const DomainBC* bcs, int nbc, bool shell_only = false, bool phi_is_zero = false, const MultiFab* cfm = nullptr, const CfTab* cftab = nullptr);
bool abec_tail_ok(const Geometry& gF, const Layout& lF, const Geometry& gC, const Layout& lC, const AbecCoef& cF, const DomainBC* bcs, int nbc, int ncomp);
void abec_tail_solve(const Geometry& gF, const AbecCoef& cF, MultiFab& corF, const MultiFab& resF, const Geometry& gC, const AbecCoef& cC,
                     const DomainBC& bc, bool singular, double eps_rel, int maxiter, int nub, int nuf, int nu1, int nu2, double omega, int* d_iters);
bool abec_residual_reads_no_ghosts(const Geometry& g, const AbecCoef& c, const MultiFab& out, const MultiFab& phi, const MultiFab& rhs, bool restrict_form);
bool abec_resid_restrict_ok(const AbecCoef& c, const MultiFab& phi, const MultiFab& rhs);
void abec_resid_restrict(const Geometry& g, const AbecCoef& c, MultiFab& crse, const MultiFab& phi, const MultiFab& rhs);
void abec_gsrb_rb(const Geometry& g, const AbecCoef& c, const AbecSmoothPlan& p, const MultiFab& pin, MultiFab& pout, const MultiFab& rhs, double omega,
                  bool zero, const DomainBC* bcs = nullptr, int nbc = 0, const CfTab* cf = nullptr, bool acc = false);
void abec_gsrb_rb_nbr(const Geometry& g, const AbecCoef& c, const AbecSmoothPlan& p, MultiFab& pin, MultiFab& pout, const MultiFab& rhs, double omega,
                      bool zero, const DomainBC* bcs, int nbc, int sel = 0, hipStream_t on = nullptr, bool acc = false);
bool abec_gsrb_rb_ok(const Geometry& g, const AbecCoef& c, const MultiFab& phi, int nbc, const DomainBC* bcs = nullptr);
bool abec_gsrb_rb_cf_ok(const Geometry& g, const AbecCoef& c, const MultiFab& phi);
bool abec_gsrb_rb_nbr_ok(const Geometry& g, const AbecCoef& c, const MultiFab& phi, const MultiFab& rhs, int nbc, const DomainBC* bcs);
bool abec_gsrb_rb_nbr_level_ok(const Geometry& g, const Layout& l, int ncomp, bool sig_form, bool has_a, int nbc, const DomainBC* bcs);
void abec_gsrb_fused(const Geometry& g, const AbecCoef& c, const MultiFab& phi_in, MultiFab& phi_out, const MultiFab& rhs, double omega,
                     const DomainBC* bcs, int nbc);
void abec_residual(const Geometry& g, const AbecCoef& c, MultiFab& out, const MultiFab& phi, const MultiFab* rhs, double* norm_out = nullptr);
bool abec_bottom_device_ok(const Geometry& g, const Layout& l, const DomainBC* bcs, int nbc, int ncomp, bool cf = false);
void abec_bottom_solve(const Geometry& g, const AbecCoef& c, MultiFab& cor, const MultiFab& res, const DomainBC& bc, bool singular,
                       double eps_rel, int maxiter, int nub, int nuf, double omega, int* d_iters, const CfTab* cftab = nullptr);
void abec_apply_domain_bc(const Geometry& g, MultiFab& phi, const DomainBC& bc, bool inhomog, const MultiFab* bcval, int comp0 = 0, int ncomp = -1);
void abec_apply_domain_bc_percomp(const Geometry& g, MultiFab& phi, const DomainBC* bcs, int ncomp, bool inhomog, const MultiFab* bcval);
void cc_restrict(MultiFab& crse, const MultiFab& fine);
void cc_prolong_add(MultiFab& fine, const MultiFab& crse);
void face_avgdown(MultiFab& crse, const MultiFab& fine, int dir);
void abec_flux(const Geometry& g, const AbecCoef& c, const MultiFab& phi, MultiFab* const flux[3], MultiFab* const add_to[3]);
void mac_rhs(const Geometry& g, MultiFab& rhs, const MultiFab* const umac[3], const MultiFab* S);
void mac_bcoef(MultiFab* const b[3], const MultiFab& rho, int rho_comp, double scale);
void mac_divergence(const Geometry& g, MultiFab& div, const MultiFab* const umac[3]);

void godunov_extrap_vel_to_faces(const Geometry& g, const MultiFab& vel, const MultiFab* force, MultiFab* const umac[3],
                                 double dt, const BCRec* bc, bool use_forces_in_trans, int scheme = 0);
void godunov_compute_aofs(const Geometry& g, MultiFab& aofs, int acomp, const MultiFab& S, int ncomp, const MultiFab* force,
                          const MultiFab* divu, MultiFab* const umac[3], const int* iconserv, double dt, const BCRec* bc,
                          bool is_velocity, bool use_forces_in_trans, MultiFab* const edge_out[3], MultiFab* const flux_out[3], int scheme = 0);


bool nodal_residual(const Geometry& g, MultiFab& out, const MultiFab& x, const MultiFab& sig, const MultiFab* rhs, double* norm_out = nullptr);
void nodal_gs_color(const Geometry& g, MultiFab& x, const MultiFab& rhs, const MultiFab& sig, int color, const MultiFab* dmask = nullptr);
void nodal_gs_fused_pass(const Geometry& g, const MultiFab& xc, const MultiFab& xn, MultiFab& xo, const MultiFab& rhs, const MultiFab& sig, int kpar,
                         bool wrap = false, const MultiFab* dmask = nullptr, const double* csig = nullptr, int zero_flags = 0, int refl = 0,
                         int sel = 0, hipStream_t on = nullptr);
bool nodal_gsr_splits(const MultiFab& x, const MultiFab& rhs, const MultiFab* dmask);
bool nodal_gsr_applies(const MultiFab& x, const MultiFab& rhs, const MultiFab* dmask);
void nodal_zero_masked(MultiFab& mf, const MultiFab& dmask);
void nodal_build_dmask(const Geometry& g, MultiFab& dm, const MultiFab& cov, const DomainBC& bc);
bool periodic_wrap_ok(const Geometry& g, const Layout& l, int min_len);
bool nodal_wrap_or_reflect_ok(const Geometry& g, const Layout& l, const DomainBC& bc, int min_len, int* refl);
bool nodal_smooth_small(const Geometry& g, MultiFab& x, const MultiFab& rhs, const MultiFab& sig, int nsweeps);
void nodal_jacobi(const Geometry& g, MultiFab& xnew, const MultiFab& x, const MultiFab& rhs, const MultiFab& sig, const MultiFab* dmask = nullptr);
void nodal_restrict(MultiFab& crse, const MultiFab& fine);
void nodal_interp_add(MultiFab& fine, const MultiFab& crse, const MultiFab& sig_fine);
void nodal_divu(const Geometry& g, MultiFab& rhs, const MultiFab& vel, int vcomp, const DomainBC* bc);
void nodal_mknewu(const Geometry& g, MultiFab* vel, int vcomp, const MultiFab& phi, const MultiFab* sig, MultiFab* gp, bool gp_increment, double vel_scale = 1.0);

void tensor_bcoef(MultiFab& b3, const MultiFab& eta, int dir);
void tensor_extensive_flux(const Geometry& g, const MultiFab& vel, const MultiFab* const eta[3], MultiFab* const flux[3], double fac, bool add);
void tensor_cross_terms_sub(const Geometry& g, const AbecCoef& c, MultiFab& out, const MultiFab& vel, double sign, unsigned long long* normout = nullptr);
void fill_tensor_corners(const Geometry& g, MultiFab& phi, const DomainBC& bc, bool inhomog, const MultiFab* bcval, int comp0 = 0, int ncomp = -1);

void les_mut(const Geometry& g, const MultiFab& vel, int vcomp, int model, double Cs, double base, MultiFab* const mu[3]);

struct TurbTable {
    int M = 0, div_free = 1;
    std::vector<int> kxyz;
    std::vector<double> data;
    mutable int* d_kxyz = nullptr;
    mutable double* d_data = nullptr;
    ~TurbTable();
};
using TurbTableP = std::shared_ptr<const TurbTable>;
void turb_host_modes(const double problo[3], const double probhi[3], int nmodes, int mode_start, int div_free, std::vector<int>& kxyz, std::vector<double>& data);
TurbTableP turb_make_table(const Geometry& g, int nmodes, int mode_start, int div_free);
TurbTableP turb_make_table(int M, const int* kxyz, const double* data, int div_free);
void turb_force(const Geometry& g, const TurbTable& tt, double time, MultiFab& out, int ocomp);

}
```

iamr_amd/csrc/mlmg.h:

```cpp
#pragma once
#include <functional>
#include "mf.h"
#include "kernels.h"
#include <vector>
#include <memory>

namespace iamrx {

inline bool mg_stalled_at_floor(const std::vector<double>& hist, double r0, double target, bool fast)
{
    const size_t n = hist.size();
    if (n == 0 || !(hist[n - 1] <= 10.0 * target)) return false;
    if (n >= 4 && hist[n - 1] > 0.9 * hist[n - 4]) return true;
    if (!fast || n < 2) return false;
    const double last = hist[n - 1] / hist[n - 2];
    double best = 1.0, prev = r0;
    for (size_t i = 0; i + 1 < n; ++i) { if (prev > 0.0) best = std::min(best, hist[i] / prev); prev = hist[i]; }
    return last > 0.5 && best < 0.2;
}


struct MGOpts {
    int nu1 = 2, nu2 = 2, nuf = 8, nub = 0;
    int max_iters = 200;
// ... 31 lines not shown
};
CycleTimer& cycle_timer();

long mg_agglomeration_cells();
bool mg_agglomerate_level(const Layout& coarse);
bool mg_slab_level(const Geometry& g, const Layout& l, int min_width, bool slab_problem);
Geometry mg_slab_geom(const Geometry& fine);
int* mg_bottom_iters_dev();

struct MGLevel {
    Geometry g;
    LayoutP layout;
    bool slab = false;
    LayoutP virt;
    MultiFab vres;
    bool agg = false;
    LayoutP dist;
    MultiFab tmp_d;
    bool res_filled = false;
};
bool mg_coarsen_level(const MGLevel& f, const MGOpts& o, MGLevel& c);

template <class Op>
void mg_restrict_to(const MGLevel& C, MultiFab& dst, MultiFab& dist_arr, MultiFab& virt_arr, Op op)
{
    MultiFab& held = C.agg ? dist_arr : dst;
    op(C.slab ? virt_arr : held);
    if (C.slab) slab_duplicate(held, virt_arr);
    if (C.agg) gather_to_replicated(dst, dist_arr);
}
inline const MultiFab& mg_correction_of(MGLevel& C, const MultiFab& cor, int ng)
{
    if (!C.agg) return cor;
    scatter_from_replicated(C.tmp_d, cor, ng);
    return C.tmp_d;
}


struct MGStats {
    int iters = 0;
    double resnorm0 = 0, rhsnorm0 = 0, resnorm = 0;
    int bottom_iters_total = 0;
    int converged = 0;
    double vcycle_ms = 0;
    int nlevels = 0;
};

class CellMG {
public:
    CellMG(const Geometry& g, LayoutP layout, int ncomp, const DomainBC& bc, const MGOpts& o);
    void setScalars(double alpha, double beta) { m_alpha = alpha; m_beta = beta; }
    void setACoeffs(const MultiFab* a) { m_a0 = a; }
    void setBCoeffs(const MultiFab* const b[3]) { for (int d = 0; d < 3; ++d) m_b0[d] = b[d]; }
    void setBCoeffsFromCell(const MultiFab* sig, int comp, double scale) { m_sig = sig; m_sig_comp = comp; m_sig_scale = scale; }
    void setTensor(bool t) { m_tensor = t; }
    void setTensorEta(bool t) { m_tensor_eta = t; }
    void setDomainBCs(const DomainBC* bcs, int n) { m_bcn.assign(bcs, bcs + n); }
    void setCoarseFineBC(const MultiFab* crse, const Geometry& cgeom, int ratio) { m_cf = true; m_crse = crse; m_cgeom = cgeom; m_ratio = ratio; }
    void prepare();
    void prepareBoundary();
    void fillBoundaryData(MultiFab& phi);
    MGStats solve(MultiFab& phi, const MultiFab& rhs, double rtol, double atol);
    void apply(MultiFab& out, MultiFab& phi);
    void fluxes(MultiFab& phi, MultiFab* const flux[3], MultiFab* const add_to[3]);
    int nlevels() const { return (int)m_lev.size(); }
    AbecCoef coef(int l) const;
    AbecCoef smoother_coef(int l) const;
    const Geometry& geom(int l) const { return m_lev[l].g; }
    void applyBC(int l, MultiFab& phi, bool inhomog, const MultiFab* bcval, bool corners = true);
    void smooth(int l, bool skip_fill, bool cf_ghosts_current = false, bool sol_is_zero = false);
    void smooth_n(int l, int nsweeps, bool skip_first_fill, bool sol_is_zero = false, MultiFab* acc = nullptr);
    void vcycle(MGStats& st);
    MultiFab& res(int l) { return m_lev[l].res; }
    MultiFab& cor(int l) { return m_lev[l].cor; }

private:
    struct Level : MGLevel {
        MultiFab a, b[3];
        MultiFab cor, res, rescor;
        MultiFab buf;
        AbecSmoothPlan plan;
        MultiFab cfm;
        CfTab cftab;
    };
    int bicgstab(int l, MultiFab& sol, const MultiFab& rhs, double eps_rel, double eps_abs, int& niters);
    void bottom_solve(MGStats& st);
    template <class Sweep> void pingpong(MultiFab& sol, MultiFab& buf, int nsweeps, bool sol_is_zero, MultiFab* acc, Sweep sweep);
    bool tail_fused() const;
    void cf_bcval(MultiFab& bcval);
    void prepare_cf(int l);
    void subtract_mean(int l, MultiFab& mf);
    Geometry m_g;
    int m_ncomp;
    std::vector<DomainBC> m_bcn;
    MGOpts m_o;
    double m_alpha = 0.0, m_beta = 1.0;
    const MultiFab* m_a0 = nullptr;
    const MultiFab* m_b0[3] = {nullptr, nullptr, nullptr};
    bool m_buni = false;
    bool m_buni_coarse = false;
    double m_bu[3] = {0.0, 0.0, 0.0};
    const MultiFab* m_sig = nullptr;
    int m_sig_comp = 0;
    double m_sig_scale = 1.0;
    bool m_tensor = false;
    bool m_tensor_eta = false;
    bool m_singular = false;
    bool m_bottom_dev = false;
    MultiFab* m_acc = nullptr;
    bool m_acc_done = false;
    bool m_bottom_direct = false;
    const double* m_dB = nullptr;
    std::shared_ptr<double> m_dBh;
    int m_dN = 0;
    void bottom_direct_prepare();
    void bottom_direct_solve();
    double m_dd_rho = 0.0;
    int m_dd_sweeps = 0;
    bool m_nbr = false;
    MultiFab m_sig2, m_a1;
    bool m_cf = false;
    const MultiFab* m_crse = nullptr;
    Geometry m_cgeom;
    int m_ratio = 2;
    std::vector<Level> m_lev;
};

class NodalMG {
public:
    NodalMG(const Geometry& g, LayoutP layout, const DomainBC& bc, const MGOpts& o);
    void setSigma(const MultiFab& sig, int comp);
    MGStats solve(MultiFab& phi, const MultiFab& rhs, double rtol, double atol, bool rhs_is_temporary = false);
    int nlevels() const { return (int)m_lev.size(); }
    bool masked() const { return m_masked; }
    const MultiFab* dmask(int l) const { return m_lev[l].dmask(); }
    const MultiFab& sigma(int l) const { return m_lev[l].sig; }
    const Geometry& geom(int l) const { return m_lev[l].g; }
    void smooth(int l, MultiFab& x, const MultiFab& rhs, bool x_is_zero = false, bool leave_ghosts = false);
    void residual(int l, MultiFab& r, MultiFab& x, const MultiFab& b, double* norm = nullptr, bool x_filled = false);
    void vcycle(MGStats& st);
    void vcycle_correction(MultiFab& e, const MultiFab& r, MGStats& st);
    void vcycle_correction_inplace(MGStats& st);
    MultiFab& res(int l) { return m_lev[l].res; }
    MultiFab& cor(int l) { return m_lev[l].cor; }

private:
    struct Level : MGLevel {
        MultiFab sig;
        MultiFab cor, res, rescor;
        MultiFab tmp;
        MultiFab xb;
        MultiFab dm;
        const MultiFab* dmask() const { return dm.defined() ? &dm : nullptr; }
    };
    int bicgstab(int l, MultiFab& sol, const MultiFab& rhs, double eps_rel, double eps_abs, int& niters);
    bool bottom_on_device();
    void subtract_mean(int l, MultiFab& mf);
    void fillbc(int l, MultiFab& x, int kpar = -1, hipStream_t on = nullptr);
    Geometry m_g;
    DomainBC m_bc;
    MGOpts m_o;
    bool m_singular = true;
    bool m_csig = false;
    double m_csig_val = 0.0;
    bool m_masked = false;
    std::vector<Level> m_lev;
};

}
```

iamr_amd/csrc/nodalmg.hip:

```cpp
#include "mlmg.h"
#include "launch.h"
#include "krylov.h"
#include <chrono>
#include <cmath>
#include <cstdlib>

namespace iamrx {

void nodal_restrict(MultiFab& crse, const MultiFab& fine);
void nodal_interp_add(MultiFab& fine, const MultiFab& crse, const MultiFab& sig_fine);

static bool nodal_fused() { return tune("NODAL_FUSED", 1) != 0; }
static bool nodal_small() { return tune("NODAL_SMALL", 1) != 0; }
bool nodal_smooth_small(const Geometry& g, MultiFab& x, const MultiFab& rhs, const MultiFab& sig, int nsweeps);
bool nodal_bottom_device_ok(const Geometry& g, const Layout& l);
void nodal_bottom_solve(const Geometry& g, MultiFab& cor, const MultiFab& res, const MultiFab& sig, bool singular, double eps_rel, int maxiter,
                        int nsweeps, int nub, int nuf, int* d_iters);
bool nodal_bottom_device_ok_general(const Geometry& g, const Layout& l);
void nodal_bottom_solve_general(const Geometry& g, MultiFab& cor, const MultiFab& res, const MultiFab& sig, const MultiFab* dmask, bool singular,
                                double eps_rel, int maxiter, int nsweeps, int nub, int nuf, int* d_iters);
static long nodal_unknowns(const Geometry& g)
{
    long n = 1;
    for (int d = 0; d < 3; ++d) n *= g.domain.len(d) + (g.periodic[d] ? 0 : 1);
    return n;
}

NodalMG::NodalMG(const Geometry& g, LayoutP layout, const DomainBC& bc_in, const MGOpts& o) : m_g(g), m_bc(bc_in), m_o(o)
{
    ProfScope ps_prof_("nmg_ctor");
    for (int d = 0; d < 3; ++d) { if (m_bc.lo[d] == lo_inflow) m_bc.lo[d] = lo_neumann; if (m_bc.hi[d] == lo_inflow) m_bc.hi[d] = lo_neumann; }
    const DomainBC& bc = m_bc;
    for (int d = 0; d < 3; ++d) {
        if (!g.periodic[d])
            for (int t : {bc.lo[d], bc.hi[d]})
                if (t != lo_neumann && t != lo_dirichlet) throw Error("iamrx NodalMG: domain boundaries must be periodic, Neumann (wall / inflow) or Dirichlet (outflow)");
        m_g.half_lo[d] = (!g.periodic[d] && bc.lo[d] == lo_neumann) ? 1 : 0;
        m_g.half_hi[d] = (!g.periodic[d] && bc.hi[d] == lo_neumann) ? 1 : 0;
    }
    m_lev.resize(1);
    m_lev[0].g = m_g;
    m_lev[0].layout = std::move(layout);
    while ((int)m_lev.size() <= m_o.max_coarsening_level) {
        Level& f = m_lev.back();
        if (m_o.device_bottom && m_o.nodal_smoother == 0 && !m_o.bottom_smoother_only &&
            (nodal_bottom_device_ok(f.g, *f.layout) || nodal_bottom_device_ok_general(f.g, *f.layout))) break;
        Level c;
        if (!mg_coarsen_level(f, m_o, c)) break;
        m_lev.push_back(std::move(c));
    }
    bool need_mask = false;
    for (int d = 0; d < 3; ++d) if (!g.periodic[d] && (bc.lo[d] == lo_dirichlet || bc.hi[d] == lo_dirichlet)) need_mask = true;
    if (m_lev[0].layout->total_cells() != g.domain.npts()) need_mask = true;
    for (auto& L : m_lev) {
        if (L.agg) L.tmp_d.define(L.dist, node_type(), 1, 1);
        if (L.slab) L.vres.define(L.virt, node_type(), 1, 0);
        const int ng = nodal_fused() ? 4 : 1;
        L.sig.define(L.layout, cell_type(), 1, ng);
        L.cor.define(L.layout, node_type(), 1, ng);
        L.res.define(L.layout, node_type(), 1, ng);
        L.rescor.define(L.layout, node_type(), 1, 1);
        int refl = 0;
        const bool written_first = tune("NODAL_SKIP_FILLS", 1) != 0 && !need_mask && m_o.nodal_smoother == 0 && nodal_fused() &&
                                   nodal_wrap_or_reflect_ok(L.g, *L.layout, m_bc, 4, &refl) && nodal_gsr_applies(L.cor, L.res, nullptr);
        if (written_first) continue;
        L.sig.setVal(0.0);
        L.cor.setVal(0.0); L.res.setVal(0.0); L.rescor.setVal(0.0);
    }
    for (auto& L : m_lev) {
        if (!need_mask) break;
        MultiFab cov(L.layout, cell_type(), 1, 1);
        cov.setVal(0.0);
        mf_add_scalar(cov, 1.0, 0, 1, 0);
        cov.FillBoundary(L.g);
        const int ng = L.cor.ngrow;
        L.dm.define(L.layout, node_type(), 1, ng);
        L.dm.setVal(1.0);
        nodal_build_dmask(L.g, L.dm, cov, m_bc);
        if (L.dm.norm0(0, 1, 0) == 0.0) L.dm = MultiFab();
        else {
            m_masked = true;
            L.dm.FillBoundary(L.g);
            nodal_reflect_bc(L.g, L.dm, m_bc);
        }
    }
    if (m_masked) {
        m_singular = false;
        for (auto& L : m_lev) IAMRX_ASSERT(L.dm.defined());
    }
}

void NodalMG::setSigma(const MultiFab& sig, int comp)
{
    ProfScope ps_prof_("nmg_setsigma");
    MultiFab::Copy(m_lev[0].sig, sig, comp, 0, 1, 0);
    m_lev[0].sig.FillBoundary(m_lev[0].g);
    cc_mirror_bc(m_lev[0].g, m_lev[0].sig);
    for (size_t l = 1; l < m_lev.size(); ++l) {
        {
            Level& C = m_lev[l];
            MultiFab sd, sv;
            if (C.agg) sd.define(C.dist, cell_type(), 1, 0);
            if (C.slab) sv.define(C.virt, cell_type(), 1, 0);
            mg_restrict_to(C, C.sig, sd, sv, [&](MultiFab& target) { cc_restrict(target, m_lev[l - 1].sig); });
        }
        m_lev[l].sig.FillBoundary(m_lev[l].g);
        cc_mirror_bc(m_lev[l].g, m_lev[l].sig);
    }
    const bool csig_on = tune("NODAL_CSIG", 1) != 0;
    m_csig = false;
    if (csig_on && !m_masked) {
        double smin, smax;
        reduce_minmax(m_lev[0].sig, 0, 0, smin, smax);
        if (smax > 0.0 && smin == smax) { m_csig = true; m_csig_val = smax; }
    }
}

void NodalMG::fillbc(int l, MultiFab& x, int kpar, hipStream_t on)
{
    const int ngv[3] = {x.ngrow, x.ngrow, 1};
    x.FillBoundary(m_lev[l].g, 0, x.ncomp, ngv, kpar, on);
    nodal_reflect_bc(m_lev[l].g, x, m_bc, on);
}

void NodalMG::smooth(int l, MultiFab& x, const MultiFab& rhs, bool x_is_zero, bool leave_ghosts)
{
    Level& L = m_lev[l];
    const int zs_mode = (int)tune("NODAL_ZERO_START", 1);
    int zs_refl = 0;
    const bool zero_start = x_is_zero && m_o.nodal_smoother == 0 && nodal_fused() && zs_mode != 0 && nodal_gsr_applies(x, rhs, L.dmask()) &&
                            (zs_mode != 2 || (!L.dmask() && nodal_wrap_or_reflect_ok(L.g, *L.layout, m_bc, 4, &zs_refl)));
    if (x_is_zero && !zero_start) x.setVal(0.0);
    const MultiFab* dmk = L.dmask();
    if (!dmk && m_o.nodal_smoother == 0 && nodal_small() && nodal_smooth_small(L.g, x, rhs, L.sig, m_o.nodal_sweeps)) {
        fillbc(l, x);
        return;
    }
    if (m_o.nodal_smoother == 0 && nodal_fused()) {
        if (!L.xb.defined() || L.xb.ngrow != x.ngrow) L.xb.define(L.layout, node_type(), 1, x.ngrow);
        int refl = 0;
        const bool wrap = !dmk && nodal_wrap_or_reflect_ok(L.g, *L.layout, m_bc, 4, &refl);
        if (!wrap) {
            if (&rhs == &L.res) { if (!L.res_filled) { fillbc(l, L.res); L.res_filled = true; } }
            else fillbc(l, const_cast<MultiFab&>(rhs));
        }
        MultiFab* a = &x;
        MultiFab* b = &L.xb;
        const bool par_fill = tune("NODAL_PARITY_FILL", 1) != 0;
        auto& ctx = Context::get();
        const int ov_mode = (int)tune("HALO_OVERLAP", 1);
        bool overlap = false;
        if (!wrap && ov_mode != 0 && nodal_gsr_splits(x, rhs, dmk)) {
            const int ngv[3] = {x.ngrow, x.ngrow, 1};
            bool peers = false;
            for (int kp = -1; kp <= 1; ++kp) peers = !fill_boundary_plan(*L.layout, node_type(), x.ngrow, L.g, ngv, kp).peers.empty() || peers;
            overlap = ov_mode == 2 || peers;
        }
        auto pass = [&](MultiFab& filled, int fill_kpar, bool do_fill, const MultiFab& xc_, const MultiFab& xn_, MultiFab& xo_, int kpar, int zf) {
            const double* cs = m_csig ? &m_csig_val : nullptr;
            if (do_fill && overlap) {
                ctx.fork_side();
                nodal_gs_fused_pass(L.g, xc_, xn_, xo_, rhs, L.sig, kpar, wrap, dmk, cs, zf, refl, 1, ctx.stream);
                fillbc(l, filled, fill_kpar, ctx.side);
                nodal_gs_fused_pass(L.g, xc_, xn_, xo_, rhs, L.sig, kpar, wrap, dmk, cs, zf, refl, 2, ctx.side);
                ctx.join_side();
                return;
            }
            if (do_fill) fillbc(l, filled, fill_kpar);
            nodal_gs_fused_pass(L.g, xc_, xn_, xo_, rhs, L.sig, kpar, wrap, dmk, cs, zf, refl);
        };
        for (int ns = 0; ns < m_o.nodal_sweeps; ++ns) {
            const bool z = zero_start && ns == 0;
            pass(*a, (ns == 0 || !par_fill) ? -1 : 1, !wrap && !z, *a, *a, *b, 0, z ? 3 : 0);
            pass(*b, par_fill ? 0 : -1, !wrap, *a, *b, *b, 1, z ? 1 : 0);
            std::swap(a, b);
        }
        if (a != &x) MultiFab::Copy(x, *a, 0, 0, 1, 0);
        if (!leave_ghosts) fillbc(l, x);
        return;
    }
    for (int ns = 0; ns < m_o.nodal_sweeps; ++ns) {
        if (false) {
        } else if (m_o.nodal_smoother == 0) {
            for (int color = 0; color < 8; ++color) {
                fillbc(l, x);
                nodal_gs_color(L.g, x, rhs, L.sig, color, dmk);
            }
        } else {
            if (!L.tmp.defined()) L.tmp.define(L.layout, node_type(), 1, 1);
            fillbc(l, x);
            nodal_jacobi(L.g, L.tmp, x, rhs, L.sig, dmk);
            MultiFab::Copy(x, L.tmp, 0, 0, 1, 0);
        }
    }
    fillbc(l, x);
}

void NodalMG::residual(int l, MultiFab& r, MultiFab& x, const MultiFab& b, double* norm, bool x_filled)
{
    if (!x_filled) fillbc(l, x);
    const bool masked = (bool)m_lev[l].dmask();
    const bool have = nodal_residual(m_lev[l].g, r, x, m_lev[l].sig, &b, (norm && !masked) ? norm : nullptr);
    if (masked) nodal_zero_masked(r, m_lev[l].dm);
    if (norm && !have) *norm = r.norm0(0, 1, 0);
}

void NodalMG::subtract_mean(int l, MultiFab& mf)
{
    const Geometry& g = m_lev[l].g;
    double cnt = 1.0;
    for (int d = 0; d < 3; ++d) cnt *= (double)g.domain.len(d);
    const double s = mf.sum_unique(g, 0);
    mf_add_scalar(mf, -s / cnt, 0, 1, 0);
}

int NodalMG::bicgstab(int l, MultiFab& sol, const MultiFab& rhs, double eps_rel, double eps_abs, int& niters)
{
    Level& L = m_lev[l];
    return bottom_bicgstab(L.layout, node_type(), 1, L.g, sol, nodal_unknowns(L.g), m_o.bottom_maxiter, eps_rel, eps_abs,
                           [&](MultiFab& r) { residual(l, r, sol, rhs); },
                           [&](MultiFab& out, MultiFab& in) {
                               fillbc(l, in);
                               nodal_residual(L.g, out, in, L.sig, nullptr);
                               if (L.dmask()) nodal_zero_masked(out, L.dm);
                           }, niters);
}

bool NodalMG::bottom_on_device()
{
    Level& B = m_lev.back();
    if (!(m_o.device_bottom && m_o.nodal_smoother == 0 && !m_o.bottom_smoother_only)) return false;
    return (!B.dmask() && nodal_bottom_device_ok(B.g, *B.layout)) || nodal_bottom_device_ok_general(B.g, *B.layout);
}

void NodalMG::vcycle(MGStats& st)
{
    const int nl = (int)m_lev.size();
    for (int l = 0; l < nl - 1; ++l) {
        Level& L = m_lev[l];
        if (m_o.nodal_nu1 <= 0) L.cor.setVal(0.0);
        for (int i = 0; i < m_o.nodal_nu1; ++i) smooth(l, L.cor, L.res, i == 0);
        residual(l, L.rescor, L.cor, L.res, nullptr, m_o.nodal_nu1 > 0);
        fillbc(l, L.rescor);
        Level& C = m_lev[l + 1];
        mg_restrict_to(C, C.res, C.tmp_d, C.vres, [&](MultiFab& target) { nodal_restrict(target, L.rescor); });
        m_lev[l + 1].res_filled = false;
        if (m_lev[l + 1].dmask()) nodal_zero_masked(m_lev[l + 1].res, m_lev[l + 1].dm);
    }
    {
        const int l = nl - 1;
        Level& B = m_lev[l];
        B.cor.setVal(0.0);
        if (m_o.bottom_smoother_only) {
            for (int i = 0; i < m_o.nuf; ++i) smooth(l, B.cor, B.res);
        } else if (bottom_on_device()) {
            const int maxiter = krylov_maxiter(m_o.bottom_maxiter, nodal_unknowns(B.g));
            if (!B.dmask() && nodal_bottom_device_ok(B.g, *B.layout))
                nodal_bottom_solve(B.g, B.cor, B.res, B.sig, m_singular, m_o.bottom_reltol, maxiter, m_o.nodal_sweeps, m_o.nub, m_o.nuf,
                                   mg_bottom_iters_dev());
            else
                nodal_bottom_solve_general(B.g, B.cor, B.res, B.sig, B.dmask(), m_singular, m_o.bottom_reltol, maxiter, m_o.nodal_sweeps, m_o.nub,
                                           m_o.nuf, mg_bottom_iters_dev());
        } else {
            MultiFab rb(B.layout, node_type(), 1, 0);
            MultiFab::Copy(rb, B.res, 0, 0, 1, 0);
            if (m_singular) subtract_mean(l, rb);
            int nit = 0;
            const int ret = bicgstab(l, B.cor, rb, m_o.bottom_reltol, -1.0, nit);
            st.bottom_iters_total += nit;
            if (ret != 0) {
                B.cor.setVal(0.0);
                for (int i = 0; i < m_o.nuf; ++i) smooth(l, B.cor, B.res);
            }
            const int nn = ret == 0 ? m_o.nub : m_o.nuf;
            for (int i = 0; i < nn; ++i) smooth(l, B.cor, B.res);
        }
    }
    for (int l = nl - 2; l >= 0; --l) {
        Level& L = m_lev[l];
        if (l + 1 == nl - 1 || m_o.nodal_nu2 <= 0) fillbc(l + 1, m_lev[l + 1].cor);
        nodal_interp_add(L.cor, mg_correction_of(m_lev[l + 1], m_lev[l + 1].cor, 1), L.sig);
        if (L.dmask()) nodal_zero_masked(L.cor, L.dm);
        for (int i = 0; i < m_o.nodal_nu2; ++i) smooth(l, L.cor, L.res, false, l == 0 && i == m_o.nodal_nu2 - 1);
    }
}

void NodalMG::vcycle_correction(MultiFab& e, const MultiFab& r, MGStats& st)
{
    Level& L0 = m_lev[0];
    MultiFab::Copy(L0.res, r, 0, 0, 1, 0);
    if (L0.dmask()) nodal_zero_masked(L0.res, L0.dm);
    if (m_singular) subtract_mean(0, L0.res);
    L0.res_filled = false;
    vcycle(st);
    MultiFab::Copy(e, L0.cor, 0, 0, 1, 0);
    e.FillBoundary(L0.g);
    nodal_reflect_bc(L0.g, e, m_bc);
}

void NodalMG::vcycle_correction_inplace(MGStats& st)
{
    Level& L0 = m_lev[0];
    if (L0.dmask()) nodal_zero_masked(L0.res, L0.dm);
    if (m_singular) subtract_mean(0, L0.res);
    L0.res_filled = false;
    vcycle(st);
    const int ngv[3] = {1, 1, 1};
    L0.cor.FillBoundary(L0.g, 0, 1, ngv, -1);
    nodal_reflect_bc(L0.g, L0.cor, m_bc);
}

MGStats NodalMG::solve(MultiFab& phi, const MultiFab& rhs_in, double rtol, double atol, bool rhs_is_temporary)
{
    ProfScope ps_prof_("nmg_solve");
    auto& ctx = Context::get();
    MGStats st;
    st.nlevels = (int)m_lev.size();
    Level& L0 = m_lev[0];
    const bool inplace = rhs_is_temporary && tune("NODAL_RHS_INPLACE", 1) != 0;
    MultiFab rhs_copy;
    if (!inplace) {
        rhs_copy.define(L0.layout, node_type(), 1, 0);
        MultiFab::Copy(rhs_copy, rhs_in, 0, 0, 1, 0);
    }
    MultiFab& rhs = inplace ? const_cast<MultiFab&>(rhs_in) : rhs_copy;
    if (L0.dmask()) nodal_zero_masked(rhs, L0.dm);
    if (m_singular) subtract_mean(0, rhs);
    residual(0, L0.res, phi, rhs, &st.resnorm0);
    L0.res_filled = false;
    st.rhsnorm0 = rhs.norm0(0, 1, 0);
    const double max_norm = st.rhsnorm0 >= st.resnorm0 ? st.rhsnorm0 : st.resnorm0;
    if (!std::isfinite(max_norm)) throw Error("iamrx nodal MLMG: the right-hand side or the initial residual is not finite");
    const double res_target = std::max(atol, std::max(rtol, 1.e-16) * max_norm);
    st.resnorm = st.resnorm0;
    if (m_o.verbose) printf("iamrx nodal MLMG: rhs %.6e resid0 %.6e levels %d (fused sweep %d, single-workgroup coarse smoother %d, ghost width %d)\n",
                            st.rhsnorm0, st.resnorm0, st.nlevels, (int)nodal_fused(), (int)nodal_small(), L0.cor.ngrow);
    double vc_ms = 0.0;
    cycle_timer().used = 0;
    const bool bdev = bottom_on_device();
    if (bdev) IAMRX_HIP_CHECK(hipMemsetAsync(mg_bottom_iters_dev(), 0, sizeof(int), ctx.stream));
    if (m_o.fixed_iters <= 0 && st.resnorm0 <= res_target) st.converged = 1;
    else {
        const int maxit = m_o.fixed_iters > 0 ? m_o.fixed_iters : m_o.max_iters;
        std::vector<double> hist;
        for (int iter = 0; iter < maxit; ++iter) {
            const bool all_per = L0.g.periodic[0] && L0.g.periodic[1] && L0.g.periodic[2] && !L0.dmask();
            if (m_singular && (!all_per || tune("MG_RES_MEAN", 0) != 0)) { subtract_mean(0, L0.res); L0.res_filled = false; }
            cycle_timer().mark(ctx.stream);
            vcycle(st);
            cycle_timer().mark(ctx.stream);
            mf_saxpy(phi, 1.0, L0.cor, 0, 0, 1, 0);
            residual(0, L0.res, phi, rhs, &st.resnorm);
            L0.res_filled = false;
            st.iters = iter + 1;
            if (m_o.verbose) printf("iamrx nodal MLMG: iter %d resid %.6e\n", iter + 1, st.resnorm);
            if (m_o.fixed_iters <= 0 && st.resnorm <= res_target) { st.converged = 1; break; }
            if (!(st.resnorm < 1.e20 * max_norm)) throw Error("iamrx nodal MLMG: failing to converge (residual blow-up)");
            hist.push_back(st.resnorm);
            if (m_o.fixed_iters <= 0 && mg_stalled_at_floor(hist, st.resnorm0, res_target, tune("MG_STALL_FAST", 1) != 0)) {
                st.converged = 2;
                fprintf(stderr, "iamrx nodal MLMG: WARNING: residual %.3e stalled at the round-off floor above the target %.3e after %d cycles; accepted (converged = 2)\n",
                        st.resnorm, res_target, st.iters);
                break;
            }
        }
        if (m_o.fixed_iters <= 0 && !st.converged) throw Error("iamrx nodal MLMG: failed to converge after max_iters");
    }
    vc_ms = cycle_timer().total_ms();
    if (st.iters > 0) st.vcycle_ms = vc_ms / st.iters;
    if (bdev && st.iters > 0) {
        int h = 0;
        IAMRX_HIP_CHECK(hipMemcpyAsync(&h, mg_bottom_iters_dev(), sizeof(int), hipMemcpyDeviceToHost, ctx.stream));
        ctx.sync();
        st.bottom_iters_total = h;
    }
    fillbc(0, phi);
    return st;
}

}
```

iamr_amd/ns.py:

```python
import ctypes as C
from .lib import lib, check, i3, mg_opts, MgStats, MultiFab, _h


class NsParams(C.Structure):
    _fields_ = [("cfl", C.c_double), ("visc_coef", C.c_double), ("be_cn_theta", C.c_double), ("gravity", C.c_double),
                ("mac_tol", C.c_double), ("mac_abs_tol", C.c_double), ("proj_tol", C.c_double),
                ("proj_abs_tol", C.c_double), ("visc_tol", C.c_double),
                ("use_forces_in_trans", C.c_int), ("do_mom_diff", C.c_int), ("init_iter", C.c_int),
                ("init_vel_iter", C.c_int), ("init_shrink", C.c_double), ("change_max", C.c_double),
                ("fixed_dt", C.c_double), ("nscal", C.c_int), ("verbose", C.c_int),
                ("init_dt", C.c_double), ("tracer_diff_coef", C.c_double), ("phys_lo", C.c_int * 3), ("phys_hi", C.c_int * 3),
                ("wall_vel_lo", C.c_double * 9), ("wall_vel_hi", C.c_double * 9),
                ("scal_bc_lo", C.c_double * 12), ("scal_bc_hi", C.c_double * 12), ("do_cons_trac", C.c_int), ("do_denminmax", C.c_int), ("do_scalminmax", C.c_int),
                ("do_trac2", C.c_int), ("do_cons_trac2", C.c_int), ("tracer2_diff_coef", C.c_double), ("do_temp", C.c_int), ("temp_cond_coef", C.c_double), ("use_ppm", C.c_int),
                ("avg_interval", C.c_int), ("compute_fluctuations", C.c_int), ("sum_interval", C.c_int),
                ("do_LES", C.c_int), ("LES_model", C.c_int), ("smago_Cs_cst", C.c_double), ("sigma_Cs_cst", C.c_double)]


def ns_params(**kw):
    p = NsParams()
    lib().iamrx_ns_default_params(C.byref(p))
    p.avg_in_checkpoint = int(kw.pop("avg_in_checkpoint", 1))
    p.turb_forcing, p.turb_nmodes = int(kw.pop("turb_forcing", 0)), int(kw.pop("turb_nmodes", 4))
    p.turb_mode_start, p.turb_div_free = int(kw.pop("turb_mode_start", 0)), int(kw.pop("turb_div_free", 1))
    for k, v in kw.items():
        if k in ("phys_lo", "phys_hi"):
            setattr(p, k, (C.c_int * 3)(*[int(x) for x in v]))
        elif k in ("wall_vel_lo", "wall_vel_hi"):
            setattr(p, k, (C.c_double * 9)(*[float(x) for x in v]))
        elif k in ("scal_bc_lo", "scal_bc_hi"):
            v = [float(x) for x in v]
            if len(v) == 6:
                v = [v[2 * d + n] if n < 2 else 0.0 for d in range(3) for n in range(4)]
            setattr(p, k, (C.c_double * 12)(*v))
        else:
            setattr(p, k, v)
    return p


def nodal_residual(geom, out, phi, sig, rhs=None):
    check(lib().iamrx_nodal_residual(C.byref(geom), out.h, phi.h, sig.h, _h(rhs)))


def nodal_gs_color(geom, phi, rhs, sig, color):
    check(lib().iamrx_nodal_gs_color(C.byref(geom), phi.h, rhs.h, sig.h, color))


def nodal_gs_sweep(geom, phi, rhs, sig, fused=1):
    check(lib().iamrx_nodal_gs_sweep(C.byref(geom), phi.h, rhs.h, sig.h, int(fused)))


def nodal_restrict(crse, fine):
    check(lib().iamrx_nodal_restrict(crse.h, fine.h))


def nodal_interp_add(fine, crse, sig_fine):
    check(lib().iamrx_nodal_interp_add(fine.h, crse.h, sig_fine.h))


def nodal_divu(geom, rhs, vel, vcomp=0, lobc=None, hibc=None):
    if lobc is None and hibc is None:
        check(lib().iamrx_nodal_divu(C.byref(geom), rhs.h, vel.h, vcomp))
    else:
        check(lib().iamrx_nodal_divu_bc(C.byref(geom), rhs.h, vel.h, vcomp, i3(lobc), i3(hibc)))


def nodal_compgrad(geom, gp, phi):
    check(lib().iamrx_nodal_compgrad(C.byref(geom), gp.h, phi.h))


def nodal_solve(geom, phi, rhs, sig, sig_comp=0, lobc=(0, 0, 0), hibc=(0, 0, 0), rel_tol=1e-12, abs_tol=1e-16, opts=None):
    st = MgStats()
    o = opts if opts is not None else mg_opts()
    check(lib().iamrx_nodal_solve(C.byref(geom), _h(phi), _h(rhs), _h(sig), sig_comp, i3(lobc), i3(hibc),
                                      C.c_double(rel_tol), C.c_double(abs_tol), C.byref(o), C.byref(st)))
    return st


def nodal_projection(geom, vel, vcomp, phi, sig, sig_comp=0, lobc=(0, 0, 0), hibc=(0, 0, 0), rel_tol=1e-12, abs_tol=1e-16,
                     opts=None, gp=None, increment_gp=False):
    st = MgStats()
    o = opts if opts is not None else mg_opts()
    check(lib().iamrx_nodal_projection(C.byref(geom), vel.h, vcomp, phi.h, sig.h, sig_comp, i3(lobc), i3(hibc),
                                       C.c_double(rel_tol), C.c_double(abs_tol), C.byref(o), _h(gp), int(increment_gp), C.byref(st)))
    return st


def _bcn(lobc, hibc):
    if hasattr(lobc[0], "__len__"):
        flat_lo = [int(v) for c in lobc for v in c]
        flat_hi = [int(v) for c in hibc for v in c]
        return (C.c_int * 9)(*flat_lo), (C.c_int * 9)(*flat_hi), 3
    return i3(lobc), i3(hibc), 1


def tensor_apply(geom, out, vel, a, b, acoef, eta, lobc=(0, 0, 0), hibc=(0, 0, 0), maxorder=2):
    lo, hi, nbc = _bcn(lobc, hibc)
    check(lib().iamrx_tensor_apply(C.byref(geom), out.h, vel.h, C.c_double(a), C.c_double(b), _h(acoef), eta[0].h, eta[1].h,
                                   eta[2].h, lo, hi, nbc, maxorder))


def tensor_solve(geom, soln, rhs, a, b, acoef, eta, lobc=(0, 0, 0), hibc=(0, 0, 0), tol_rel=1e-10, tol_abs=0.0, opts=None):
    st = MgStats()
    o = opts if opts is not None else mg_opts(maxorder=2)
    lo, hi, nbc = _bcn(lobc, hibc)
    check(lib().iamrx_tensor_solve(C.byref(geom), soln.h, rhs.h, C.c_double(a), C.c_double(b), _h(acoef), eta[0].h, eta[1].h,
                                   eta[2].h, lo, hi, nbc, C.c_double(tol_rel), C.c_double(tol_abs), C.byref(o), C.byref(st)))
    return st


def tensor_apply_cf(geom, out, vel, a, b, acoef, eta, crse_vel, cgeom, ratio=2, lobc=(0, 0, 0), hibc=(0, 0, 0), maxorder=2):
    lo, hi, nbc = _bcn(lobc, hibc)
    check(lib().iamrx_tensor_apply_cf(C.byref(geom), out.h, vel.h, C.c_double(a), C.c_double(b), _h(acoef), eta[0].h, eta[1].h,
                                      eta[2].h, lo, hi, nbc, maxorder, _h(crse_vel), C.byref(cgeom), int(ratio)))


def tensor_solve_cf(geom, soln, rhs, a, b, acoef, eta, crse_vel, cgeom, ratio=2, lobc=(0, 0, 0), hibc=(0, 0, 0), tol_rel=1e-10, tol_abs=0.0,
                    opts=None):
    st = MgStats()
    o = opts if opts is not None else mg_opts(maxorder=2)
    lo, hi, nbc = _bcn(lobc, hibc)
    check(lib().iamrx_tensor_solve_cf(C.byref(geom), soln.h, rhs.h, C.c_double(a), C.c_double(b), _h(acoef), eta[0].h, eta[1].h,
                                      eta[2].h, lo, hi, nbc, _h(crse_vel), C.byref(cgeom), int(ratio), C.c_double(tol_rel), C.c_double(tol_abs),
                                      C.byref(o), C.byref(st)))
    return st


SMAGORINSKY, SIGMA = 0, 1


def les_mut(geom, vel, mu, model, Cs, base=0.0, vcomp=0):
    check(lib().iamrx_les_mut(C.byref(geom), vel.h, int(vcomp), int(model), C.c_double(Cs), C.c_double(base), mu[0].h, mu[1].h, mu[2].h))


def calc_mut_les(geom, vel, mu, model, Cs, lobc=((0, 0, 0),) * 3, hibc=((0, 0, 0),) * 3, maxorder=3, crse_vel=None, cgeom=None, ratio=2):
    lo, hi, nbc = _bcn(lobc, hibc)
    assert nbc == 3
    if cgeom is None:
        check(lib().iamrx_calc_mut_les(C.byref(geom), vel.h, lo, hi, int(maxorder), int(model), C.c_double(Cs), mu[0].h, mu[1].h, mu[2].h))
    else:
        check(lib().iamrx_calc_mut_les_cf(C.byref(geom), vel.h, lo, hi, int(maxorder), int(model), C.c_double(Cs), mu[0].h, mu[1].h, mu[2].h,
                                          _h(crse_vel), C.byref(cgeom), int(ratio)))


class NavierStokes:
    S_NEW, S_OLD, P_NEW, P_OLD, GP_NEW, GP_OLD, UMAC_X, UMAC_Y, UMAC_Z, AOFS = range(10)
    ETA_N, ETA_NP1 = 13, 16
    AVERAGE = 12
    VEL_AVG_NAMES = ["x_vel_average", "y_vel_average", "z_vel_average", "x_vel_rms", "y_vel_rms", "z_vel_rms"]
    _types = {0: ((0, 0, 0), 5, 1), 1: ((0, 0, 0), 5, 1), 2: ((1, 1, 1), 1, 1), 3: ((1, 1, 1), 1, 1), 4: ((0, 0, 0), 3, 1),
              5: ((0, 0, 0), 3, 1), 6: ((1, 0, 0), 1, 1), 7: ((0, 1, 0), 1, 1), 8: ((0, 0, 1), 1, 1), 9: ((0, 0, 0), 5, 0),
              12: ((0, 0, 0), 6, 0), 13: ((1, 0, 0), 1, 0), 14: ((0, 1, 0), 1, 0), 15: ((0, 0, 1), 1, 0), 16: ((1, 0, 0), 1, 0),
              17: ((0, 1, 0), 1, 0), 18: ((0, 0, 1), 1, 0)}

    def __init__(self, geom, layout, params=None, opts=None):
        self.geom = geom
        self.layout = layout
        self.params = params if params is not None else ns_params()
        self.opts = opts if opts is not None else mg_opts()
        self.h = C.c_void_p()
        check(lib().iamrx_ns_create(C.byref(geom), layout.h, C.byref(self.params), C.byref(self.opts), C.byref(self.h)))
        if getattr(self.params, "turb_forcing", 0):
            self.set_turb_forcing(self.params.turb_nmodes, self.params.turb_mode_start, self.params.turb_div_free)

    def set_turb_forcing(self, nmodes=4, mode_start=0, div_free=1, on=1):
        check(lib().iamrx_ns_set_turb_forcing(self.h, int(on), int(nmodes), int(mode_start), int(div_free)))

    def init_rayleightaylor(self, rho_1, rho_2, tra_1=0.0, tra_2=0.0, pertamp=0.0, interface_width=1.0):
        check(lib().iamrx_ns_init_rayleightaylor(self.h, C.c_double(rho_1), C.c_double(rho_2), C.c_double(tra_1), C.c_double(tra_2),
                                                 C.c_double(pertamp), C.c_double(interface_width)))

    def init_taylorgreen(self, vfac=1.0, a=1.0, b=1.0, c=0.0, rho0=1.0):
        check(lib().iamrx_ns_init_taylorgreen(self.h, C.c_double(vfac), C.c_double(a), C.c_double(b), C.c_double(c), C.c_double(rho0)))

    def init_rest(self, rho0=1.0):
        check(lib().iamrx_ns_init_rest(self.h, C.c_double(rho0)))

    def set_turb_modes(self, kxyz, data, div_free=1):
        from .lib import _turb_table
        M, k, d = _turb_table(kxyz, data)
        check(lib().iamrx_ns_set_turb_modes(self.h, M, k, d, int(div_free)))

    def set_data(self, which, mf):
        check(lib().iamrx_ns_set_data(self.h, int(which), mf.h))

    def post_init(self, stop_time=-1.0):
        check(lib().iamrx_ns_post_init(self.h, C.c_double(stop_time)))

    def step(self):
        dt = C.c_double()
        check(lib().iamrx_ns_step(self.h, C.byref(dt)))
        return dt.value

    def advance(self, dt):
        est = C.c_double()
        check(lib().iamrx_ns_advance(self.h, C.c_double(dt), C.byref(est)))
        return est.value

    @property
    def time(self):
        t = C.c_double()
        check(lib().iamrx_ns_time(self.h, C.byref(t), None, None))
        return t.value

    @property
    def dt(self):
# ... 61 lines not shown
```

include/iamrx.h:

```cpp
#ifndef IAMRX_H
#define IAMRX_H
#include <stddef.h>

#ifdef __cplusplus
extern "C" {
#endif

typedef struct iamrx_layout_s* iamrx_layout;
typedef struct iamrx_fluxreg_s* iamrx_fluxreg;
typedef struct iamrx_mf_s* iamrx_mf;
typedef struct iamrx_ns_s* iamrx_ns;
typedef struct iamrx_syncreg_s* iamrx_syncreg;
typedef struct iamrx_amr_s* iamrx_amr;

typedef struct iamrx_geom {
    int dom_lo[3], dom_hi[3];
    double prob_lo[3], prob_hi[3];
    int periodic[3];
} iamrx_geom;

typedef struct iamrx_mg_opts {
    int nu1, nu2, nuf, nub;
    int max_iters, bottom_maxiter;
    double bottom_reltol;
    double omega;
    int maxorder;
    int max_coarsening_level, min_width;
    int nodal_sweeps, nodal_smoother;
    int verbose;
    int bottom_smoother_only;
    int fixed_iters;
    int nodal_nu1, nodal_nu2;
    int device_bottom;
    int slab;
} iamrx_mg_opts;

typedef struct iamrx_mg_stats {
    int iters;
    double resnorm0, rhsnorm0, resnorm;
    int bottom_iters_total;
    int converged;
    double vcycle_ms;
    int nlevels;
} iamrx_mg_stats;

int iamrx_init(int device);
int iamrx_finalize(void);
const char* iamrx_last_error(void);
int iamrx_sync(void);
void* iamrx_stream(void);
int iamrx_mem_info(size_t* bytes_live, size_t* bytes_cached);
int iamrx_alloc_count(size_t* n_device_malloc);
int iamrx_tuning_set(const char* key, double value);
int iamrx_tuning_get(const char* key, double default_value, double* value);
int iamrx_scope_profile(int enable, int reset, char* report, size_t capacity);
int iamrx_exchange_counts(size_t out[4]);
int iamrx_coalesce_merge_count(size_t* n);
int iamrx_sync_count(size_t* n_stream_sync);
int iamrx_timer_start(void);
int iamrx_timer_stop(double* ms);
void iamrx_mg_default_opts(iamrx_mg_opts* o);
int iamrx_kernel_probe_start(int which, long min_points, int stride);
int iamrx_kernel_probe_stop(int which, double* total_ms, long* launches);

int iamrx_comm_get_unique_id(char id[128]);
int iamrx_comm_init_rccl(const char id[128], int rank, int nranks);
typedef void (*iamrx_allreduce_cb)(double* vals, int n, int op);
typedef void (*iamrx_exchange_cb)(int nsend, const int* send_peers, double** send_bufs, const long* send_counts,
                                  int nrecv, const int* recv_peers, double** recv_bufs, const long* recv_counts);
int iamrx_comm_init_callback(int rank, int nranks, iamrx_allreduce_cb ar, iamrx_exchange_cb ex);
int iamrx_comm_rank(int* rank, int* nranks);
int iamrx_comm_allreduce(double* vals, int n, int op);
int iamrx_comm_probe_exchange(int peer, long count);
const char* iamrx_comm_last_error(void);

int iamrx_layout_create(int nboxes, const int* lo_hi , const int* owner_rank,
                        iamrx_layout* out);
int iamrx_layout_coalesced_boxes(iamrx_layout l, int* nboxes, int* lo_hi );
int iamrx_layout_destroy(iamrx_layout l);
int iamrx_layout_nlocal(iamrx_layout l, int* nlocal);
int iamrx_layout_local_box(iamrx_layout l, int local_idx, int lo_hi[6], int* global_idx);
int iamrx_layout_owners(iamrx_layout l, int* owners );
int iamrx_mf_create(iamrx_layout l, const int type[3] , int ncomp, int ngrow, iamrx_mf* out);
int iamrx_mf_destroy(iamrx_mf m);
int iamrx_mf_info(iamrx_mf m, int* ncomp, int* ngrow, int type[3], int* nlocal);
int iamrx_mf_fab_box(iamrx_mf m, int local_idx, int lo_hi[6]);
int iamrx_mf_dev_ptr(iamrx_mf m, int local_idx, double** p);
int iamrx_mf_to_host(iamrx_mf m, int local_idx, double* dst);
int iamrx_mf_from_host(iamrx_mf m, int local_idx, const double* src);
int iamrx_mf_setval(iamrx_mf m, double v);
int iamrx_mf_copy(iamrx_mf dst, iamrx_mf src, int scomp, int dcomp, int ncomp, int ngrow);
int iamrx_mf_fill_boundary(iamrx_mf m, const iamrx_geom* g);
int iamrx_mf_fill_physbc(iamrx_mf m, const iamrx_geom* g, int scomp, int ncomp, const int* bcrec, const double* extdir_lo,
                         const double* extdir_hi);
int iamrx_mf_norm0(iamrx_mf m, int comp, int ncomp, int ngrow, double* out);
int iamrx_mf_norm0_comps(iamrx_mf m, int comp, int ncomp, int ngrow, int form, double* out);
int iamrx_mf_minmax(iamrx_mf m, int comp, int ngrow, double* mn, double* mx);
int iamrx_mf_dot(const iamrx_geom* g, const int lobc[3], const int hibc[3], iamrx_mf x0, iamrx_mf y0, iamrx_mf x1, iamrx_mf y1, int comp,
                 int ncomp, int on_device, double out[2]);
int iamrx_mf_sum_unique(const iamrx_geom* g, const int lobc[3], const int hibc[3], iamrx_mf m, int comp, double* out);

int iamrx_host_fill_plan(int nboxes, const int* lo_hi, const int* owner, int rank, const int type[3], int ngrow, const iamrx_geom* g,
                         int max_desc, int* desc, int* ndesc);
int iamrx_host_fill_plan_wall_ext(int nboxes, const int* lo_hi, const int* owner, int rank, const int type[3], int ngrow, const iamrx_geom* g,
                                  int wall_ext, int max_desc, int* desc, int* ndesc);

int iamrx_host_abec_smoother_plan(int nboxes, const int* lo_hi, const iamrx_geom* g, const int lobc[3], const int hibc[3], int maxorder, int ncomp,
                                  int coef, int has_a, int has_cf, int finest, const int ngrow[4], int out[12]);

int iamrx_abec_gsrb(const iamrx_geom* g, double alpha, double beta, iamrx_mf a , iamrx_mf bx, iamrx_mf by, iamrx_mf bz,
                    iamrx_mf phi, iamrx_mf rhs, int redblack, double omega, const int lobc[3], const int hibc[3], int maxorder);
int iamrx_abec_form(const iamrx_geom* g, int coef, iamrx_mf rho, int rho_comp, double scale, const double bu[3], double beta, int op,
                    iamrx_mf phi, iamrx_mf rhs, iamrx_mf out, double omega, const int lobc[3], const int hibc[3], int maxorder);
int iamrx_abec_gsrb_sweep(const iamrx_geom* g, double alpha, double beta, iamrx_mf a , iamrx_mf bx, iamrx_mf by, iamrx_mf bz,
                          iamrx_mf phi, iamrx_mf rhs, double omega, const int lobc[3], const int hibc[3], int maxorder, int fused);
int iamrx_abec_residual(const iamrx_geom* g, double alpha, double beta, iamrx_mf a, iamrx_mf bx, iamrx_mf by, iamrx_mf bz,
                        iamrx_mf out, iamrx_mf phi, iamrx_mf rhs, int tensor);
int iamrx_cc_restrict(iamrx_mf crse, iamrx_mf fine);
int iamrx_cc_prolong_add(iamrx_mf fine, iamrx_mf crse);
int iamrx_face_avgdown(iamrx_mf crse, iamrx_mf fine, int dir);
int iamrx_abec_solve(const iamrx_geom* g, double alpha, double beta, iamrx_mf a, iamrx_mf bx, iamrx_mf by, iamrx_mf bz,
                     iamrx_mf phi, iamrx_mf rhs, const int lobc[3], const int hibc[3], double rtol, double atol,
                     const iamrx_mg_opts* o, int tensor, iamrx_mg_stats* st);

int iamrx_mlmg_mac_solve(const iamrx_geom* g, iamrx_mf umac_x, iamrx_mf umac_y, iamrx_mf umac_z, iamrx_mf rho, int rho_comp,
                         iamrx_mf S , iamrx_mf mac_phi, double rhs_scale, const int lobc[3], const int hibc[3],
                         double mac_tol, double mac_abs_tol, const iamrx_mg_opts* o, iamrx_mg_stats* st);
int iamrx_mlmg_mac_solve_cf(const iamrx_geom* g, iamrx_mf umac_x, iamrx_mf umac_y, iamrx_mf umac_z, iamrx_mf rho, int rho_comp,
                            iamrx_mf S , iamrx_mf mac_phi, double rhs_scale, const int lobc[3], const int hibc[3],
                            iamrx_mf crse_phi, const iamrx_geom* cgeom, int ratio, double mac_tol, double mac_abs_tol,
                            const iamrx_mg_opts* o, iamrx_mg_stats* st);
int iamrx_mac_sync_solve(const iamrx_geom* g, iamrx_fluxreg mac_reg, iamrx_mf rho_half, double dt, iamrx_layout fine, int ratio,
                         iamrx_mf ucorr_x, iamrx_mf ucorr_y, iamrx_mf ucorr_z, iamrx_mf mac_sync_phi, const int lobc[3], const int hibc[3],
                         double mac_sync_tol, double mac_abs_tol, const iamrx_mg_opts* o, iamrx_mg_stats* st);
int iamrx_mac_divergence(const iamrx_geom* g, iamrx_mf div, iamrx_mf umac_x, iamrx_mf umac_y, iamrx_mf umac_z);

#define IAMRX_GODUNOV_PLM 0
#define IAMRX_GODUNOV_PPM 1
#define IAMRX_BDS 2
int iamrx_godunov_extrap_vel_to_faces(const iamrx_geom* g, iamrx_mf vel, iamrx_mf force, iamrx_mf umac_x, iamrx_mf umac_y,
                                      iamrx_mf umac_z, double dt, const int* bcrec , int use_forces_in_trans, int scheme);
int iamrx_godunov_compute_aofs(const iamrx_geom* g, iamrx_mf aofs, int acomp, iamrx_mf S, int ncomp, iamrx_mf force, iamrx_mf divu,
                               iamrx_mf umac_x, iamrx_mf umac_y, iamrx_mf umac_z, const int* iconserv, double dt,
                               const int* bcrec , int is_velocity, int use_forces_in_trans,
                               iamrx_mf edge_x, iamrx_mf edge_y, iamrx_mf edge_z, iamrx_mf flux_x, iamrx_mf flux_y, iamrx_mf flux_z, int scheme);

int iamrx_nodal_residual(const iamrx_geom* g, iamrx_mf out, iamrx_mf phi, iamrx_mf sig, iamrx_mf rhs);
int iamrx_nodal_gs_color(const iamrx_geom* g, iamrx_mf phi, iamrx_mf rhs, iamrx_mf sig, int color);
int iamrx_nodal_gs_sweep(const iamrx_geom* g, iamrx_mf phi, iamrx_mf rhs, iamrx_mf sig, int fused);
int iamrx_nodal_restrict(iamrx_mf crse, iamrx_mf fine);
int iamrx_nodal_interp_add(iamrx_mf fine, iamrx_mf crse, iamrx_mf sig_fine);
int iamrx_nodal_divu(const iamrx_geom* g, iamrx_mf rhs, iamrx_mf vel, int vcomp);
int iamrx_nodal_divu_bc(const iamrx_geom* g, iamrx_mf rhs, iamrx_mf vel, int vcomp, const int lobc[3], const int hibc[3]);
int iamrx_nodal_compgrad(const iamrx_geom* g, iamrx_mf gp, iamrx_mf phi);
int iamrx_nodal_projection(const iamrx_geom* g, iamrx_mf vel, int vcomp, iamrx_mf phi, iamrx_mf sig, int sig_comp,
                           const int lobc[3], const int hibc[3], double rel_tol, double abs_tol, const iamrx_mg_opts* o,
                           iamrx_mf gp , int increment_gp, iamrx_mg_stats* st);

int iamrx_abec_solve_cf(const iamrx_geom* g, double alpha, double beta, iamrx_mf a, iamrx_mf bx, iamrx_mf by, iamrx_mf bz,
                        iamrx_mf phi, iamrx_mf rhs, const int lobc[3], const int hibc[3], iamrx_mf crse_phi, const iamrx_geom* cgeom,
                        int ratio, double rel_tol, double abs_tol, const iamrx_mg_opts* o, iamrx_mg_stats* st);

int iamrx_nodal_solve(const iamrx_geom* g, iamrx_mf phi, iamrx_mf rhs, iamrx_mf sig, int sig_comp, const int lobc[3], const int hibc[3],
                      double rel_tol, double abs_tol, const iamrx_mg_opts* o, iamrx_mg_stats* st);

int iamrx_tensor_apply(const iamrx_geom* g, iamrx_mf out, iamrx_mf vel, double a, double b, iamrx_mf acoef, iamrx_mf eta_x,
                       iamrx_mf eta_y, iamrx_mf eta_z, const int* lobc, const int* hibc, int nbc, int maxorder);
int iamrx_tensor_solve(const iamrx_geom* g, iamrx_mf soln, iamrx_mf rhs, double a, double b, iamrx_mf acoef, iamrx_mf eta_x,
                       iamrx_mf eta_y, iamrx_mf eta_z, const int* lobc, const int* hibc, int nbc, double tol_rel, double tol_abs,
                       const iamrx_mg_opts* o, iamrx_mg_stats* st);

int iamrx_tensor_extensive_flux(const iamrx_geom* g, iamrx_mf vel, iamrx_mf eta_x, iamrx_mf eta_y, iamrx_mf eta_z,
                                iamrx_mf flux_x, iamrx_mf flux_y, iamrx_mf flux_z, double fac, int add);
int iamrx_tensor_apply_cf(const iamrx_geom* g, iamrx_mf out, iamrx_mf vel, double a, double b, iamrx_mf acoef, iamrx_mf eta_x,
                          iamrx_mf eta_y, iamrx_mf eta_z, const int* lobc, const int* hibc, int nbc, int maxorder,
                          iamrx_mf crse_vel, const iamrx_geom* cgeom, int ratio);
int iamrx_tensor_solve_cf(const iamrx_geom* g, iamrx_mf soln, iamrx_mf rhs, double a, double b, iamrx_mf acoef, iamrx_mf eta_x,
                          iamrx_mf eta_y, iamrx_mf eta_z, const int* lobc, const int* hibc, int nbc, iamrx_mf crse_vel,
                          const iamrx_geom* cgeom, int ratio, double tol_rel, double tol_abs, const iamrx_mg_opts* o, iamrx_mg_stats* st);

int iamrx_les_mut(const iamrx_geom* g, iamrx_mf vel, int vcomp, int model, double Cs, double base, iamrx_mf mu_x, iamrx_mf mu_y, iamrx_mf mu_z);

int iamrx_host_turb_modes(const double prob_lo[3], const double prob_hi[3], int nmodes, int mode_start, int div_free, int cap, int* M, int* kxyz, double* data);
int iamrx_turb_force(const iamrx_geom* g, int M, const int* kxyz, const double* data, int div_free, double time, iamrx_mf out, int ocomp);
int iamrx_calc_mut_les(const iamrx_geom* g, iamrx_mf vel, const int* lobc, const int* hibc, int maxorder, int model, double Cs,
                       iamrx_mf mu_x, iamrx_mf mu_y, iamrx_mf mu_z);
int iamrx_calc_mut_les_cf(const iamrx_geom* g, iamrx_mf vel, const int* lobc, const int* hibc, int maxorder, int model, double Cs,
                          iamrx_mf mu_x, iamrx_mf mu_y, iamrx_mf mu_z, iamrx_mf crse_vel, const iamrx_geom* cgeom, int ratio);

int iamrx_parallel_copy(iamrx_mf dst, iamrx_mf src, int scomp, int dcomp, int ncomp, int src_ng, int dst_ng, const iamrx_geom* periodic_geom);
int iamrx_average_down(iamrx_mf fine, iamrx_mf crse, int scomp, int ncomp, int ratio);
int iamrx_create_umac_grown(iamrx_mf umac_fine_x, iamrx_mf umac_fine_y, iamrx_mf umac_fine_z, iamrx_mf umac_crse_x, iamrx_mf umac_crse_y,
                            iamrx_mf umac_crse_z, iamrx_mf divu, const iamrx_geom* cgeom, const iamrx_geom* fgeom, int ratio);
int iamrx_fluxreg_create(iamrx_layout fine, iamrx_layout crse, const iamrx_geom* cgeom, int ratio, int ncomp, iamrx_fluxreg* out);
int iamrx_fluxreg_destroy(iamrx_fluxreg fr);
int iamrx_fluxreg_setval(iamrx_fluxreg fr, double v);
int iamrx_fluxreg_crse_init(iamrx_fluxreg fr, iamrx_mf crse_flux, int dir, int scomp, int dcomp, int ncomp, double mult, int add);
int iamrx_fluxreg_fine_add(iamrx_fluxreg fr, iamrx_mf fine_flux, int dir, int scomp, int dcomp, int ncomp, double mult);
int iamrx_fluxreg_reflux(iamrx_fluxreg fr, iamrx_mf S_crse, double volume, double scale, int scomp, int dcomp, int ncomp);
int iamrx_fillpatch_two_levels(iamrx_mf dst, int dcomp, double time, iamrx_mf fine_old, iamrx_mf fine_new, double t_fine_old, double t_fine_new,
                               iamrx_mf crse_old, iamrx_mf crse_new, double t_crse_old, double t_crse_new, int scomp, int ncomp,
                               const iamrx_geom* cgeom, const iamrx_geom* fgeom, int ratio, const int* bcrec, const double* extdir_lo, const double* extdir_hi);

int iamrx_derive_mag_vort(const iamrx_geom* g, iamrx_mf out, int ocomp, iamrx_mf vel, int vcomp);
int iamrx_error_tag(const iamrx_geom* g, iamrx_mf tags, iamrx_mf field, int comp, int mode, double value, int level,
                    const double* realbox_lo, const double* realbox_hi);
int iamrx_cluster_tags(const iamrx_geom* g, iamrx_mf tags, int blocking_factor, int max_grid_size, double grid_eff, int n_error_buf,
                       int* boxes, int* nboxes);
int iamrx_host_cluster_tags(const unsigned char* tags, const int dom_lo[3], const int dom_hi[3], int blocking_factor, int max_grid_size, double grid_eff,
                            int n_error_buf, const unsigned char* allowed, int* boxes, int* nboxes);
int iamrx_host_erode(unsigned char* map, const int n[3], const int periodic[3], int passes);

typedef struct iamrx_diffusion_crse { iamrx_mf crse_old, crse_new; const iamrx_geom* cgeom; int ratio; } iamrx_diffusion_crse;
int iamrx_diffuse_scalar(const iamrx_geom* g, iamrx_mf S_old, iamrx_mf Rho_old, iamrx_mf S_new, iamrx_mf Rho_new, int sigma, int rho_comp, double dt,
                         double be_cn_theta, iamrx_mf rho_half, int rho_flag, const iamrx_mf* fluxn, const iamrx_mf* fluxnp1, iamrx_mf delta_rhs,
                         int rhs_comp, const iamrx_mf* betan, const iamrx_mf* betanp1, const int* lobc, const int* hibc,
                         const iamrx_diffusion_crse* crse, int add_old_time_divFlux, double visc_tol, const iamrx_mg_opts* o, iamrx_mg_stats* st);
int iamrx_diffuse_tensor_velocity(const iamrx_geom* g, iamrx_mf U_old, iamrx_mf U_new, int rho_comp, double dt, double be_cn_theta, iamrx_mf rho_half,
                                  int rho_flag, iamrx_mf visc_old_term, const iamrx_mf* eta_n, const iamrx_mf* eta_np1, const int* lobc, const int* hibc,
                                  const iamrx_diffusion_crse* crse, const iamrx_mf* tflux, double visc_tol, const iamrx_mg_opts* o, iamrx_mg_stats* st,
                                  void (*fill_new)(void* ctx, iamrx_mf U_new), void* ctx);
int iamrx_diffuse_tensor_vsync(const iamrx_geom* g, iamrx_mf Vsync, double dt, double be_cn_theta, iamrx_mf rho_half, int rho_flag, iamrx_mf Rho_old,
                               iamrx_mf Rho_new, int rho_comp, const iamrx_mf* eta, const int* lobc, const int* hibc, const int* bcrec_vel,
                               const iamrx_geom* cgeom, int ratio, const iamrx_mf* tflux, double visc_tol, const iamrx_mg_opts* o, iamrx_mg_stats* st);
int iamrx_diffuse_ssync(const iamrx_geom* g, iamrx_mf Ssync, int comp, double dt, double be_cn_theta, iamrx_mf rho_half, int rho_flag, iamrx_mf Rho_new,
                        int rho_comp, const iamrx_mf* beta, const int* lobc, const int* hibc, const iamrx_geom* cgeom, int ratio, const iamrx_mf* flux,
                        double visc_tol, const iamrx_mg_opts* o, iamrx_mg_stats* st);

typedef struct iamrx_ns_params {
    double cfl, visc_coef, be_cn_theta, gravity;
    double mac_tol, mac_abs_tol, proj_tol, proj_abs_tol, visc_tol;
    int use_forces_in_trans, do_mom_diff, init_iter, init_vel_iter;
    double init_shrink, change_max, fixed_dt;
    int nscal, verbose;
    double init_dt;
    double tracer_diff_coef;
    int phys_lo[3], phys_hi[3];
    double wall_vel_lo[9], wall_vel_hi[9];
    double scal_bc_lo[12], scal_bc_hi[12];
    int do_cons_trac;
    int do_denminmax, do_scalminmax;
    int do_trac2, do_cons_trac2;
    double tracer2_diff_coef;
    int do_temp;
    double temp_cond_coef;
    int use_ppm;
    int avg_interval;
    int compute_fluctuations;
    int sum_interval;
    int do_LES;
    int LES_model;
    double smago_Cs_cst;
    double sigma_Cs_cst;
} iamrx_ns_params;
void iamrx_ns_default_params(iamrx_ns_params* p);
int iamrx_ns_create(const iamrx_geom* g, iamrx_layout l, const iamrx_ns_params* p, const iamrx_mg_opts* o, iamrx_ns* out);
int iamrx_ns_destroy(iamrx_ns ns);
int iamrx_ns_set_turb_forcing(iamrx_ns ns, int on, int nmodes, int mode_start, int div_free);
int iamrx_ns_set_turb_modes(iamrx_ns ns, int M, const int* kxyz, const double* data, int div_free);
int iamrx_ns_init_taylorgreen(iamrx_ns ns, double vfac, double a, double b, double c, double rho0);
int iamrx_ns_init_rayleightaylor(iamrx_ns ns, double rho_1, double rho_2, double tra_1, double tra_2, double pertamp, double interface_width);
int iamrx_ns_init_rest(iamrx_ns ns, double rho0);
int iamrx_ns_post_init(iamrx_ns ns, double stop_time);
int iamrx_ns_step(iamrx_ns ns, double* dt_used);
int iamrx_ns_advance(iamrx_ns ns, double dt, double* dt_est);
int iamrx_ns_time(iamrx_ns ns, double* time, double* dt, int* nstep);
int iamrx_ns_data(iamrx_ns ns, int which, iamrx_mf* out);
int iamrx_ns_derive(iamrx_ns ns, const char* name, iamrx_mf out, int ocomp);
int iamrx_ns_time_average(iamrx_ns ns, double dt_level, int level0_steps);
int iamrx_ns_average_state(iamrx_ns ns, int set, double v[3]);
int iamrx_ns_sum_integrated(iamrx_ns ns, double sums[3]);

int iamrx_ns_set_data(iamrx_ns ns, int which, iamrx_mf src);
int iamrx_ns_restart_state(iamrx_ns ns, int set, double state[16]);
int iamrx_ns_stats(iamrx_ns ns, iamrx_mg_stats* mac, iamrx_mg_stats* nodal, iamrx_mg_stats* visc);
int iamrx_ns_profile(iamrx_ns ns, int enable, double sections_ms[8]);

int iamrx_mf_alias(iamrx_layout l, const int type[3], int ncomp, int ngrow, double* const* dev_ptrs, iamrx_mf* out);

int iamrx_level_project(const iamrx_geom* g, double dt, iamrx_mf U_new, int vcomp, iamrx_mf P_new, iamrx_mf Gp_old, iamrx_mf Gp_new,
                        iamrx_mf rho_half, const int lobc[3], const int hibc[3], double proj_tol, double proj_abs_tol,
                        const iamrx_mg_opts* o, iamrx_mg_stats* st);

int iamrx_syncreg_create(iamrx_layout fine, iamrx_layout crse, const iamrx_geom* cgeom, const iamrx_geom* fgeom, int ratio,
                         const int phys_lo[3], const int phys_hi[3], iamrx_syncreg* out);
int iamrx_syncreg_destroy(iamrx_syncreg r);
int iamrx_syncreg_crse_init(iamrx_syncreg r, iamrx_mf sync_resid_crse, double mult);
int iamrx_syncreg_fine_add(iamrx_syncreg r, iamrx_mf sync_resid_fine, double mult);
int iamrx_syncreg_init_rhs(iamrx_syncreg r, iamrx_mf rhs);
typedef struct iamrx_proj_level { const iamrx_geom* geom; iamrx_layout layout; int lobc[3], hibc[3]; int ratio; iamrx_mf gp; } iamrx_proj_level;
int iamrx_mlsync_project(const iamrx_proj_level* crse, const iamrx_proj_level* fine, iamrx_mf pres_crse, iamrx_mf vel_crse, int vcomp_crse, iamrx_mf pres_fine,
                         iamrx_mf vel_fine, int vcomp_fine, iamrx_mf rho_crse, iamrx_mf rho_fine, iamrx_mf Vsync, iamrx_mf V_corr, iamrx_mf phi_crse,
                         iamrx_mf phi_fine, iamrx_syncreg rhs_sync_reg, iamrx_syncreg crse_sync_reg, double dt, int crse_iteration, int crse_dt_ratio,
                         double sync_tol, double abs_tol, const iamrx_mg_opts* o, iamrx_mg_stats* st);
int iamrx_sync_interp(iamrx_mf fine_dst, int dcomp, iamrx_mf crse_sync, int scomp, int ncomp, const iamrx_geom* cgeom, const iamrx_geom* fgeom,
                      int ratio, const int* bcrec );
int iamrx_godunov_compute_aofs_sync(const iamrx_geom* g, iamrx_mf sync, int acomp, iamrx_mf S, int ncomp, iamrx_mf force, iamrx_mf divu,
                                    iamrx_mf umac_x, iamrx_mf umac_y, iamrx_mf umac_z, iamrx_mf ucorr_x, iamrx_mf ucorr_y, iamrx_mf ucorr_z,
                                    const int* iconserv, double dt, const int* bcrec, int is_velocity, int use_forces_in_trans,
                                    iamrx_mf flux_x, iamrx_mf flux_y, iamrx_mf flux_z, int scheme);

int iamrx_syncreg_comp_add(iamrx_syncreg r, iamrx_mf sync_resid_fine, const iamrx_geom* fgeom, iamrx_layout finer, int finer_ratio, double mult);
int iamrx_mac_sync_compute(const iamrx_geom* g, iamrx_mf ucorr_x, iamrx_mf ucorr_y, iamrx_mf ucorr_z, iamrx_mf Vsync, iamrx_mf Ssync, iamrx_mf S_vel,
// ... 50 lines not shown
```

Before: 486.0 million cells/s.

## Read periodic/reflect images directly in nodal residual and restrict, skipping ghost fills

Nodal residual and restriction kernels now map out-of-box indices to their periodic or reflected images when the level is a single box spanning a periodic or Neumann domain. The nodal multigrid then skips the fillbc ghost exchanges before residual, restriction and after smoothing on such levels. This removes several ghost-fill kernel launches and copies per V-cycle, at the cost of extra index arithmetic in the kernels. It also retunes the residual kernel's k-chunk size for single-box layouts so more blocks launch.

```diff
diff --git a/iamr_amd/csrc/cabi.hip b/iamr_amd/csrc/cabi.hip
--- a/iamr_amd/csrc/cabi.hip
+++ b/iamr_amd/csrc/cabi.hip
@@ -628,6 +628,30 @@
 {
     IAMRX_TRY nodal_residual(to_geom(g), out->mf, phi->mf, sig->mf, rhs ? &rhs->mf : nullptr); IAMRX_CATCH
 }
+static NodalImages images_of(const Geometry& g, const MultiFab& mf, const int lobc[3], const int hibc[3], const char* who)
+{
+    NodalImages img;
+    img.on = nodal_wrap_or_reflect_ok(g, *mf.layout, to_bc(lobc, hibc, 2), 4, &img.refl);
+    if (!img.on) throw Error(std::string(who) + ": the level is not one box of at least 4 cells per direction spanning a domain that is periodic or ends on Neumann walls");
+    return img;
+}
+int iamrx_nodal_residual_images(const iamrx_geom* g, iamrx_mf out, iamrx_mf phi, iamrx_mf sig, iamrx_mf rhs, const int lobc[3], const int hibc[3],
+                                double* norm)
+{
+    IAMRX_TRY
+    const Geometry gg = to_geom(g);
+    const NodalImages img = images_of(gg, phi->mf, lobc, hibc, "iamrx_nodal_residual_images");
+    if (!nodal_residual(gg, out->mf, phi->mf, sig->mf, rhs ? &rhs->mf : nullptr, norm, img) && norm) *norm = out->mf.norm0(0, 1, 0);
+    IAMRX_CATCH
+}
+int iamrx_nodal_restrict_images(const iamrx_geom* g, iamrx_mf c, iamrx_mf f, const int lobc[3], const int hibc[3])
+{
+    IAMRX_TRY
+    const NodalImages img = images_of(to_geom(g), f->mf, lobc, hibc, "iamrx_nodal_restrict_images");
+    if (c->mf.layout->boxes.size() != 1 || c->mf.nlocal() != 1) throw Error("iamrx_nodal_restrict_images: the coarse level is not one box");
+    nodal_restrict(c->mf, f->mf, img);
+    IAMRX_CATCH
+}
 int iamrx_nodal_gs_color(const iamrx_geom* g, iamrx_mf phi, iamrx_mf rhs, iamrx_mf sig, int color)
 {
     IAMRX_TRY nodal_gs_color(to_geom(g), phi->mf, rhs->mf, sig->mf, color); IAMRX_CATCH
diff --git a/iamr_amd/csrc/k_nodal.hip b/iamr_amd/csrc/k_nodal.hip
--- a/iamr_amd/csrc/k_nodal.hip
+++ b/iamr_amd/csrc/k_nodal.hip
@@ -38,8 +38,47 @@
     y += w.fz * (x(i, j, k - 1) * (smmm + spmm + smpm + sppm) + x(i, j, k + 1) * (smmp + spmp + smpp + sppp));
     return y;
 }
-
-void nodal_residual_launch(const Geometry& g, MultiFab& out, const MultiFab& x, const MultiFab& sig, const MultiFab* rhs, unsigned long long* d_norm);
+__device__ __forceinline__ double node_Ax_at(const FabD& x, const FabD& s, const NodeW& w, int im, int i, int ip, int jm, int j, int jp, int km, int k, int kp,
+                                             double& s0)
+{
+    const double smmm = s(i - 1, j - 1, k - 1), spmm = s(i, j - 1, k - 1), smpm = s(i - 1, j, k - 1), sppm = s(i, j, k - 1);
+    const double smmp = s(i - 1, j - 1, k), spmp = s(i, j - 1, k), smpp = s(i - 1, j, k), sppp = s(i, j, k);
+    s0 = w.c * (smmm + spmm + smpm + sppm + smmp + spmp + smpp + sppp);
+    double y = x(i, j, k) * s0;
+    y += w.corner * (x(im, jm, km) * smmm + x(ip, jm, km) * spmm + x(im, jp, km) * smpm + x(ip, jp, km) * sppm
+                   + x(im, jm, kp) * smmp + x(ip, jm, kp) * spmp + x(im, jp, kp) * smpp + x(ip, jp, kp) * sppp);
+    y += w.ex * (x(i, jm, km) * (smmm + spmm) + x(i, jp, km) * (smpm + sppm) + x(i, jm, kp) * (smmp + spmp) + x(i, jp, kp) * (smpp + sppp));
+    y += w.ey * (x(im, j, km) * (smmm + smpm) + x(ip, j, km) * (spmm + sppm) + x(im, j, kp) * (smmp + smpp) + x(ip, j, kp) * (spmp + sppp));
+    y += w.ez * (x(im, jm, k) * (smmm + smmp) + x(ip, jm, k) * (spmm + spmp) + x(im, jp, k) * (smpm + smpp) + x(ip, jp, k) * (sppm + sppp));
+    y += w.fx * (x(im, j, k) * (smmm + smpm + smmp + smpp) + x(ip, j, k) * (spmm + sppm + spmp + sppp));
+    y += w.fy * (x(i, jm, k) * (smmm + spmm + smmp + spmp) + x(i, jp, k) * (smpm + sppm + smpp + sppp));
+    y += w.fz * (x(i, j, km) * (smmm + spmm + smpm + sppm) + x(i, j, kp) * (smmp + spmp + smpp + sppp));
+    return y;
+}
+
+__device__ __forceinline__ int wrap_node(int g, int lo, int hi)
+{
+    const int n = hi - lo + 1;
+    return g < lo ? g + n : (g > hi + 1 ? g - n : g);
+}
+__device__ __forceinline__ int wrap_cell(int g, int lo, int hi)
+{
+    const int n = hi - lo + 1;
+    return g < lo ? g + n : (g > hi ? g - n : g);
+}
+__device__ __forceinline__ int image_node(int g, int lo, int hi, bool refl)
+{
+    if (refl) return g < lo ? 2 * lo - g : (g > hi + 1 ? 2 * (hi + 1) - g : g);
+    return wrap_node(g, lo, hi);
+}
+__device__ __forceinline__ int image_cell(int g, int lo, int hi, bool refl)
+{
+    if (refl) return g < lo ? 2 * lo - 1 - g : (g > hi ? 2 * hi + 1 - g : g);
+    return wrap_cell(g, lo, hi);
+}
+
+void nodal_residual_launch(const Geometry& g, MultiFab& out, const MultiFab& x, const MultiFab& sig, const MultiFab* rhs, unsigned long long* d_norm,
+                           const NodalImages& img);
 __device__ __forceinline__ void nodal_norm_commit(double mx, unsigned long long* out)
 {
     for (int o = 32; o > 0; o >>= 1) mx = fmax(mx, __shfl_xor(mx, o, 64));
@@ -51,7 +90,7 @@
 template <int TX, int TY>
 __global__ void __launch_bounds__(TX * TY) k_nodal_residual_zm(const BoxD* __restrict__ boxes, const FabD* __restrict__ ot, const FabD* __restrict__ xt,
     const FabD* __restrict__ st, const FabD* __restrict__ rt, NodeW w, int ntx, int nty, int kc, unsigned long long* __restrict__ normout,
-    const int4* __restrict__ list)
+    const int4* __restrict__ list, int images, int refl)
 {
     double mx = 0.0;
     constexpr int RX = TX + 2, RY = TY + 2, NT = TX * TY, NLD = (RX * RY + NT - 1) / NT;
@@ -75,7 +114,8 @@
         const int idx = min(tid + it * NT, RX * RY - 1);
         lidx[it] = idx;
         const int gi = ox + idx % RX, gj = oy + idx / RX;
-        const int xi = min(max(gi, x.lo[0]), x.lo[0] + x.n[0] - 1), xj = min(max(gj, x.lo[1]), x.lo[1] + x.n[1] - 1);
+        const int mi = images ? image_node(gi, cb.lo[0], cb.hi[0], refl & 1) : gi, mj = images ? image_node(gj, cb.lo[1], cb.hi[1], refl & 2) : gj;
+        const int xi = min(max(mi, x.lo[0]), x.lo[0] + x.n[0] - 1), xj = min(max(mj, x.lo[1]), x.lo[1] + x.n[1] - 1);
         const int si = min(max(gi, s.lo[0]), s.lo[0] + s.n[0] - 1), sj = min(max(gj, s.lo[1]), s.lo[1] + s.n[1] - 1);
         xoff[it] = x.off(xi, xj, x.lo[2]);
         soff[it] = s.off(si, sj, s.lo[2]);
@@ -83,7 +123,7 @@
     const long xpl = (long)x.n[0] * x.n[1], spl = (long)s.n[0] * s.n[1];
     const FabD::gdouble* xp = (const FabD::gdouble*)x.p;
     const FabD::gdouble* sp = (const FabD::gdouble*)s.p;
-    auto ldx = [&](int it, int k) { return xp[xoff[it] + xpl * (k - x.lo[2])]; };
+    auto ldx = [&](int it, int k) { return xp[xoff[it] + xpl * ((images ? image_node(k, cb.lo[2], cb.hi[2], refl & 4) : k) - x.lo[2])]; };
     auto lds_ = [&](int it, int k) { return sp[soff[it] + spl * (k - s.lo[2])]; };
 #pragma unroll
     for (int it = 0; it < NLD; ++it) {
@@ -134,7 +174,7 @@
     if (normout) nodal_norm_commit(mx, normout);
 }
 
-bool nodal_residual(const Geometry& g, MultiFab& out, const MultiFab& x, const MultiFab& sig, const MultiFab* rhs, double* norm_out)
+bool nodal_residual(const Geometry& g, MultiFab& out, const MultiFab& x, const MultiFab& sig, const MultiFab* rhs, double* norm_out, const NodalImages& img)
 {
     auto& ctx = Context::get();
     static unsigned long long* d_norm = nullptr;
@@ -143,7 +183,7 @@
     const bool zm = tune("NODAL_RES_ZM", 1) != 0 && lay.max_len[0] >= 16 && lay.max_len[1] >= 8 && x.ngrow >= 1 && sig.ngrow >= 1;
     const bool fused = norm_out && zm && tune("NODAL_RES_NORM", 1) != 0;
     if (fused) IAMRX_HIP_CHECK(hipMemsetAsync(d_norm, 0, sizeof(unsigned long long), ctx.stream));
-    nodal_residual_launch(g, out, x, sig, rhs, fused ? d_norm : nullptr);
+    nodal_residual_launch(g, out, x, sig, rhs, fused ? d_norm : nullptr, img);
     if (!fused) return false;
     const bool global = !lay.replicated && ctx.comm->nranks > 1;
     if (global) ctx.comm->allreduce_device(reinterpret_cast<double*>(d_norm), 1, ReduceOp::Max, ctx.stream);
@@ -156,9 +196,11 @@
     return true;
 }
 
-void nodal_residual_launch(const Geometry& g, MultiFab& out, const MultiFab& x, const MultiFab& sig, const MultiFab* rhs, unsigned long long* d_norm)
+void nodal_residual_launch(const Geometry& g, MultiFab& out, const MultiFab& x, const MultiFab& sig, const MultiFab* rhs, unsigned long long* d_norm,
+                           const NodalImages& img)
 {
     if (x.nlocal() == 0) return;
+    IAMRX_ASSERT(!img.on || (x.layout->boxes.size() == 1 && x.nlocal() == 1));
     const NodeW w = make_w(g);
     const FabD *ot = out.d_tab, *xt = x.d_tab, *st = sig.d_tab;
     const FabD* rt = rhs ? rhs->d_tab : nullptr;
@@ -168,8 +210,15 @@
         constexpr int TX = 32, TY = 8;
         const int ntx = (l.max_len[0] + 1 + TX - 1) / TX, nty = (l.max_len[1] + 1 + TY - 1) / TY;
         const int nk = l.max_len[2] + 1;
-        const int kc = nk >= 128 ? 32 : (nk >= 32 ? 16 : nk);
+        const int kc_set = (int)tune("NODAL_RES_KC", 0);
+        int kc = nk >= 128 ? 32 : (nk >= 32 ? 16 : nk);
+        if (l.boxes.size() == 1) {
+            const long fit = (long)ntx * nty * nk / 2048;
+            while (kc > 2 && kc > fit) kc = (kc & (kc - 1)) ? (1 << (31 - __builtin_clz((unsigned)kc))) : kc / 2;
+        }
+        if (kc_set > 0) kc = std::min(kc_set, nk);
         const int nck = (nk + kc - 1) / kc;
+        const int images = img.on ? 1 : 0, refl = img.refl;
         if (l.nlocal() >= 4 && tune("TILE_LISTS", 1) != 0) {
             int n = 0;
             const int4* lst = layout_int4_list(l, {3, TX, TY, kc, 0}, [&](std::vector<int4>& h) {
@@ -181,13 +230,25 @@
             }, &n);
             if (lst && 4L * n <= 3L * ntx * nty * nck * l.nlocal()) {
                 hipLaunchKernelGGL((k_nodal_residual_zm<TX, TY>), dim3((unsigned)n), dim3(TX * TY), 0, Context::get().stream, l.d_boxes, ot, xt, st, rt, w, ntx, nty, kc,
-                                   d_norm, lst);
+                                   d_norm, lst, images, refl);
                 return;
             }
         }
         dim3 grid((unsigned)(ntx * nty * nck), (unsigned)l.nlocal());
         hipLaunchKernelGGL((k_nodal_residual_zm<TX, TY>), grid, dim3(TX * TY), 0, Context::get().stream, l.d_boxes, ot, xt, st, rt, w, ntx, nty, kc, d_norm,
-                           (const int4*)nullptr);
+                           (const int4*)nullptr, images, refl);
+        return;
+    }
+    if (img.on) {
+        const BoxD b = l.boxes[0];
+        const int refl = img.refl;
+        for_each(*x.layout, node_type(), 0, Context::get().stream, [=] __device__(int i, int j, int k, int f) {
+            double s0;
+            const double y = node_Ax_at(xt[f], st[f], w, image_node(i - 1, b.lo[0], b.hi[0], refl & 1), i, image_node(i + 1, b.lo[0], b.hi[0], refl & 1),
+                                        image_node(j - 1, b.lo[1], b.hi[1], refl & 2), j, image_node(j + 1, b.lo[1], b.hi[1], refl & 2),
+                                        image_node(k - 1, b.lo[2], b.hi[2], refl & 4), k, image_node(k + 1, b.lo[2], b.hi[2], refl & 4), s0);
+            ot[f](i, j, k) = rt ? rt[f](i, j, k) - y : y;
+        });
         return;
     }
     for_each(*x.layout, node_type(), 0, Context::get().stream, [=] __device__(int i, int j, int k, int f) {
@@ -232,27 +293,6 @@
     Tiling t = make_tiling(ml, l.nlocal(), 4);
     hipLaunchKernelGGL(k_nodal_gscolor, t.grid(), Tiling::block(), 0, Context::get().stream, t, l.d_boxes, x.d_tab, rhs.d_tab, sig.d_tab, make_w(g), color,
                        dmask ? dmask->d_tab : nullptr);
-}
-
-__device__ __forceinline__ int wrap_node(int g, int lo, int hi)
-{
-    const int n = hi - lo + 1;
-    return g < lo ? g + n : (g > hi + 1 ? g - n : g);
-}
-__device__ __forceinline__ int wrap_cell(int g, int lo, int hi)
-{
-    const int n = hi - lo + 1;
-    return g < lo ? g + n : (g > hi ? g - n : g);
-}
-__device__ __forceinline__ int image_node(int g, int lo, int hi, bool refl)
-{
-    if (refl) return g < lo ? 2 * lo - g : (g > hi + 1 ? 2 * (hi + 1) - g : g);
-    return wrap_node(g, lo, hi);
-}
-__device__ __forceinline__ int image_cell(int g, int lo, int hi, bool refl)
-{
-    if (refl) return g < lo ? 2 * lo - 1 - g : (g > hi ? 2 * hi + 1 - g : g);
-    return wrap_cell(g, lo, hi);
 }
 
 template <int TX, int TY, int NT, bool WRAP, bool MASK, bool CSIG>
@@ -1408,7 +1448,7 @@
 
 template <int CTX, int CTY>
 __global__ void __launch_bounds__(CTX * CTY) k_nodal_restrict_tile(const BoxD* __restrict__ cboxes, const FabD* __restrict__ ct, const FabD* __restrict__ ft,
-    int ntx, int nty, int kc)
+    int ntx, int nty, int kc, int images, int refl, BoxD fb)
 {
     constexpr int FX = 2 * CTX + 1, FY = 2 * CTY + 1, HX = CTX + 1, PX = 2 * HX, NT = CTX * CTY, NLD = (FX * FY + NT - 1) / NT;
     __shared__ double F[3][FY][PX];
@@ -1430,15 +1470,19 @@
     for (int it = 0; it < NLD; ++it) {
         const int idx = tid + it * NT;
         const int lx = idx % FX, ly = idx / FX;
-        const int gi = ox + lx, gj = oy + ly;
-        const bool on = idx < FX * FY && gi >= fa.lo[0] && gi <= fhi0 && gj >= fa.lo[1] && gj <= fhi1;
+        const bool in_reach = ox + lx <= 2 * nhi0 + 1 && oy + ly <= 2 * nhi1 + 1;
+        const int gi = images ? image_node(ox + lx, fb.lo[0], fb.hi[0], refl & 1) : ox + lx, gj = images ? image_node(oy + ly, fb.lo[1], fb.hi[1], refl & 2) : oy + ly;
+        const bool on = idx < FX * FY && in_reach && gi >= fa.lo[0] && gi <= fhi0 && gj >= fa.lo[1] && gj <= fhi1;
         foff[it] = on ? fa.off(gi, gj, fa.lo[2]) : -1;
         lslot[it] = idx < FX * FY ? ly * PX + (lx & 1) * HX + (lx >> 1) : -1;
     }
     const long fpl = (long)fa.n[0] * fa.n[1];
     const FabD::gdouble* fp = (const FabD::gdouble*)fa.p;
     const int fklo = fa.lo[2], fkhi = fa.lo[2] + fa.n[2] - 1;
-    auto ldf = [&](int it, int k) { return (foff[it] >= 0 && k >= fklo && k <= fkhi) ? (double)fp[foff[it] + fpl * (k - fklo)] : 0.0; };
+    auto ldf = [&](int it, int k_) {
+        const int k = images ? image_node(k_, fb.lo[2], fb.hi[2], refl & 4) : k_;
+        return (foff[it] >= 0 && k >= fklo && k <= fkhi) ? (double)fp[foff[it] + fpl * (k - fklo)] : 0.0;
+    };
     double* Fl = &F[0][0][0];
     constexpr int PL = FY * PX;
     int sm = 0, s0 = 1, sp = 2;
@@ -1482,9 +1526,12 @@
     }
 }
 
-void nodal_restrict(MultiFab& crse, const MultiFab& fine)
+void nodal_restrict(MultiFab& crse, const MultiFab& fine, const NodalImages& img)
 {
     if (crse.nlocal() == 0) return;
+    IAMRX_ASSERT(!img.on || (fine.layout->boxes.size() == 1 && fine.nlocal() == 1 && crse.nlocal() == 1));
+    const BoxD fb = fine.layout->boxes[0];
+    const int images = img.on ? 1 : 0, refl = img.refl;
     const FabD *ct = crse.d_tab, *ft = fine.d_tab;
     const Layout& cl = *crse.layout;
     const int min_x = std::max(16, (int)tune("NODAL_RESTRICT_MIN", 48));
@@ -1495,7 +1542,7 @@
         const int kc = nk >= 64 ? 8 : 4;
         const int nck = (nk + kc - 1) / kc;
         dim3 grid((unsigned)(ntx * nty * nck), (unsigned)cl.nlocal());
-        hipLaunchKernelGGL((k_nodal_restrict_tile<CTX, CTY>), grid, dim3(CTX * CTY), 0, Context::get().stream, cl.d_boxes, ct, ft, ntx, nty, kc);
+        hipLaunchKernelGGL((k_nodal_restrict_tile<CTX, CTY>), grid, dim3(CTX * CTY), 0, Context::get().stream, cl.d_boxes, ct, ft, ntx, nty, kc, images, refl, fb);
         return;
     }
     for_each(*crse.layout, node_type(), 0, Context::get().stream, [=] __device__(int i, int j, int k, int f) {
@@ -1506,7 +1553,9 @@
             for (int dj = -1; dj <= 1; ++dj)
                 for (int di = -1; di <= 1; ++di) {
                     const double w = (di == 0 ? 2. : 1.) * (dj == 0 ? 2. : 1.) * (dk == 0 ? 2. : 1.);
-                    s += w * fa(ii + di, jj + dj, kk + dk);
+                    int fi = ii + di, fj = jj + dj, fk = kk + dk;
+                    if (images) { fi = image_node(fi, fb.lo[0], fb.hi[0], refl & 1); fj = image_node(fj, fb.lo[1], fb.hi[1], refl & 2); fk = image_node(fk, fb.lo[2], fb.hi[2], refl & 4); }
+                    s += w * fa(fi, fj, fk);
                 }
         ct[f](i, j, k) = s * (1. / 64.);
     });
diff --git a/iamr_amd/csrc/kernels.h b/iamr_amd/csrc/kernels.h
--- a/iamr_amd/csrc/kernels.h
+++ b/iamr_amd/csrc/kernels.h
@@ -141,7 +141,9 @@
                           bool is_velocity, bool use_forces_in_trans, MultiFab* const edge_out[3], MultiFab* const flux_out[3], int scheme = 0);
 
 
-bool nodal_residual(const Geometry& g, MultiFab& out, const MultiFab& x, const MultiFab& sig, const MultiFab* rhs, double* norm_out = nullptr);
+struct NodalImages { bool on = false; int refl = 0; };
+bool nodal_residual(const Geometry& g, MultiFab& out, const MultiFab& x, const MultiFab& sig, const MultiFab* rhs, double* norm_out = nullptr,
+                    const NodalImages& img = NodalImages());
 void nodal_gs_color(const Geometry& g, MultiFab& x, const MultiFab& rhs, const MultiFab& sig, int color, const MultiFab* dmask = nullptr);
 void nodal_gs_fused_pass(const Geometry& g, const MultiFab& xc, const MultiFab& xn, MultiFab& xo, const MultiFab& rhs, const MultiFab& sig, int kpar,
                          bool wrap = false, const MultiFab* dmask = nullptr, const double* csig = nullptr, int zero_flags = 0, int refl = 0,
@@ -154,7 +156,7 @@
 bool nodal_wrap_or_reflect_ok(const Geometry& g, const Layout& l, const DomainBC& bc, int min_len, int* refl);
 bool nodal_smooth_small(const Geometry& g, MultiFab& x, const MultiFab& rhs, const MultiFab& sig, int nsweeps);
 void nodal_jacobi(const Geometry& g, MultiFab& xnew, const MultiFab& x, const MultiFab& rhs, const MultiFab& sig, const MultiFab* dmask = nullptr);
-void nodal_restrict(MultiFab& crse, const MultiFab& fine);
+void nodal_restrict(MultiFab& crse, const MultiFab& fine, const NodalImages& img = NodalImages());
 void nodal_interp_add(MultiFab& fine, const MultiFab& crse, const MultiFab& sig_fine);
 void nodal_divu(const Geometry& g, MultiFab& rhs, const MultiFab& vel, int vcomp, const DomainBC* bc);
 void nodal_mknewu(const Geometry& g, MultiFab* vel, int vcomp, const MultiFab& phi, const MultiFab* sig, MultiFab* gp, bool gp_increment, double vel_scale = 1.0);
diff --git a/iamr_amd/csrc/mlmg.h b/iamr_amd/csrc/mlmg.h
--- a/iamr_amd/csrc/mlmg.h
+++ b/iamr_amd/csrc/mlmg.h
@@ -207,6 +207,7 @@
         MultiFab xb;
         MultiFab dm;
         const MultiFab* dmask() const { return dm.defined() ? &dm : nullptr; }
+        NodalImages img;
     };
     int bicgstab(int l, MultiFab& sol, const MultiFab& rhs, double eps_rel, double eps_abs, int& niters);
     bool bottom_on_device();
diff --git a/iamr_amd/csrc/nodalmg.hip b/iamr_amd/csrc/nodalmg.hip
--- a/iamr_amd/csrc/nodalmg.hip
+++ b/iamr_amd/csrc/nodalmg.hip
@@ -7,7 +7,6 @@
 
 namespace iamrx {
 
-void nodal_restrict(MultiFab& crse, const MultiFab& fine);
 void nodal_interp_add(MultiFab& fine, const MultiFab& crse, const MultiFab& sig_fine);
 
 static bool nodal_fused() { return tune("NODAL_FUSED", 1) != 0; }
@@ -88,6 +87,11 @@
         m_singular = false;
         for (auto& L : m_lev) IAMRX_ASSERT(L.dm.defined());
     }
+    const bool img_on = tune("NODAL_IMAGE_READERS", 1) != 0 && m_o.nodal_smoother == 0 && nodal_fused();
+    for (auto& L : m_lev) {
+        L.img.on = img_on && !L.dmask() && nodal_wrap_or_reflect_ok(L.g, *L.layout, m_bc, 4, &L.img.refl);
+        if (!L.img.on) L.img.refl = 0;
+    }
 }
 
 void NodalMG::setSigma(const MultiFab& sig, int comp)
@@ -133,7 +137,7 @@
     if (x_is_zero && !zero_start) x.setVal(0.0);
     const MultiFab* dmk = L.dmask();
     if (!dmk && m_o.nodal_smoother == 0 && nodal_small() && nodal_smooth_small(L.g, x, rhs, L.sig, m_o.nodal_sweeps)) {
-        fillbc(l, x);
+        if (!L.img.on) fillbc(l, x);
         return;
     }
     if (m_o.nodal_smoother == 0 && nodal_fused()) {
@@ -176,7 +180,7 @@
             std::swap(a, b);
         }
         if (a != &x) MultiFab::Copy(x, *a, 0, 0, 1, 0);
-        if (!leave_ghosts) fillbc(l, x);
+        if (!leave_ghosts && !L.img.on) fillbc(l, x);
         return;
     }
     for (int ns = 0; ns < m_o.nodal_sweeps; ++ns) {
@@ -198,9 +202,10 @@
 
 void NodalMG::residual(int l, MultiFab& r, MultiFab& x, const MultiFab& b, double* norm, bool x_filled)
 {
-    if (!x_filled) fillbc(l, x);
+    const NodalImages& img = m_lev[l].img;
+    if (!x_filled && !img.on) fillbc(l, x);
     const bool masked = (bool)m_lev[l].dmask();
-    const bool have = nodal_residual(m_lev[l].g, r, x, m_lev[l].sig, &b, (norm && !masked) ? norm : nullptr);
+    const bool have = nodal_residual(m_lev[l].g, r, x, m_lev[l].sig, &b, (norm && !masked) ? norm : nullptr, img);
     if (masked) nodal_zero_masked(r, m_lev[l].dm);
     if (norm && !have) *norm = r.norm0(0, 1, 0);
 }
@@ -241,9 +246,10 @@
         if (m_o.nodal_nu1 <= 0) L.cor.setVal(0.0);
         for (int i = 0; i < m_o.nodal_nu1; ++i) smooth(l, L.cor, L.res, i == 0);
         residual(l, L.rescor, L.cor, L.res, nullptr, m_o.nodal_nu1 > 0);
-        fillbc(l, L.rescor);
         Level& C = m_lev[l + 1];
-        mg_restrict_to(C, C.res, C.tmp_d, C.vres, [&](MultiFab& target) { nodal_restrict(target, L.rescor); });
+        const NodalImages rimg = (!C.slab && !C.agg) ? L.img : NodalImages();
+        if (!rimg.on) fillbc(l, L.rescor);
+        mg_restrict_to(C, C.res, C.tmp_d, C.vres, [&](MultiFab& target) { nodal_restrict(target, L.rescor, rimg); });
         m_lev[l + 1].res_filled = false;
         if (m_lev[l + 1].dmask()) nodal_zero_masked(m_lev[l + 1].res, m_lev[l + 1].dm);
     }
@@ -278,7 +284,7 @@
     }
     for (int l = nl - 2; l >= 0; --l) {
         Level& L = m_lev[l];
-        if (l + 1 == nl - 1 || m_o.nodal_nu2 <= 0) fillbc(l + 1, m_lev[l + 1].cor);
+        if ((l + 1 == nl - 1 || m_o.nodal_nu2 <= 0) && !m_lev[l + 1].img.on) fillbc(l + 1, m_lev[l + 1].cor);
         nodal_interp_add(L.cor, mg_correction_of(m_lev[l + 1], m_lev[l + 1].cor, 1), L.sig);
         if (L.dmask()) nodal_zero_masked(L.cor, L.dm);
         for (int i = 0; i < m_o.nodal_nu2; ++i) smooth(l, L.cor, L.res, false, l == 0 && i == m_o.nodal_nu2 - 1);
diff --git a/iamr_amd/ns.py b/iamr_amd/ns.py
--- a/iamr_amd/ns.py
+++ b/iamr_amd/ns.py
@@ -42,6 +42,12 @@
     check(lib().iamrx_nodal_residual(C.byref(geom), out.h, phi.h, sig.h, _h(rhs)))
 
 
+def nodal_residual_images(geom, out, phi, sig, rhs=None, lobc=(0, 0, 0), hibc=(0, 0, 0)):
+    norm = C.c_double()
+    check(lib().iamrx_nodal_residual_images(C.byref(geom), out.h, phi.h, sig.h, _h(rhs), i3(lobc), i3(hibc), C.byref(norm)))
+    return norm.value
+
+
 def nodal_gs_color(geom, phi, rhs, sig, color):
     check(lib().iamrx_nodal_gs_color(C.byref(geom), phi.h, rhs.h, sig.h, color))
 
@@ -52,6 +58,10 @@
 
 def nodal_restrict(crse, fine):
     check(lib().iamrx_nodal_restrict(crse.h, fine.h))
+
+
+def nodal_restrict_images(geom, crse, fine, lobc=(0, 0, 0), hibc=(0, 0, 0)):
+    check(lib().iamrx_nodal_restrict_images(C.byref(geom), crse.h, fine.h, i3(lobc), i3(hibc)))
 
 
 def nodal_interp_add(fine, crse, sig_fine):
diff --git a/include/iamrx.h b/include/iamrx.h
--- a/include/iamrx.h
+++ b/include/iamrx.h
@@ -146,9 +146,12 @@
                                iamrx_mf edge_x, iamrx_mf edge_y, iamrx_mf edge_z, iamrx_mf flux_x, iamrx_mf flux_y, iamrx_mf flux_z, int scheme);
 
 int iamrx_nodal_residual(const iamrx_geom* g, iamrx_mf out, iamrx_mf phi, iamrx_mf sig, iamrx_mf rhs);
+int iamrx_nodal_residual_images(const iamrx_geom* g, iamrx_mf out, iamrx_mf phi, iamrx_mf sig, iamrx_mf rhs, const int lobc[3], const int hibc[3],
+                                double* norm);
 int iamrx_nodal_gs_color(const iamrx_geom* g, iamrx_mf phi, iamrx_mf rhs, iamrx_mf sig, int color);
 int iamrx_nodal_gs_sweep(const iamrx_geom* g, iamrx_mf phi, iamrx_mf rhs, iamrx_mf sig, int fused);
 int iamrx_nodal_restrict(iamrx_mf crse, iamrx_mf fine);
+int iamrx_nodal_restrict_images(const iamrx_geom* g, iamrx_mf crse, iamrx_mf fine, const int lobc[3], const int hibc[3]);
 int iamrx_nodal_interp_add(iamrx_mf fine, iamrx_mf crse, iamrx_mf sig_fine);
 int iamrx_nodal_divu(const iamrx_geom* g, iamrx_mf rhs, iamrx_mf vel, int vcomp);
 int iamrx_nodal_divu_bc(const iamrx_geom* g, iamrx_mf rhs, iamrx_mf vel, int vcomp, const int lobc[3], const int hibc[3]);
```

After: 494.9 million cells/s (median of 6 runs). 1.02x the previous value.
